# UCLALibrary/jp2-bucketeer

Hardware: AMD Instinct MI355X
Metric: encoded megapixels/sec (node), lossless 5/3 + lossy 9/7, at 1/2/4/8 MI355X (higher is better)
Workload: dtype f32+i32

## Files before the change

jp2-bucketeer_amd/csrc/encode.cpp:

```cpp
#include <algorithm>
#include <cmath>
#include <cstddef>
#include <cstring>
#include <string>
#include <vector>

#include "context.h"
#include "encode.h"
#include "source_layout.h"

namespace jp2hip {

void default_recipe(jp2hip_recipe *r, int conversion) {
    std::memset(r, 0, sizeof *r);
    r->levels = 6;
    r->layers = 6;
    r->tile_w = r->tile_h = 512;
    r->cblk_w_log2 = r->cblk_h_log2 = 6;
    r->nprecincts = 3;
    r->prec_w_log2[0] = r->prec_h_log2[0] = 8;
    r->prec_w_log2[1] = r->prec_h_log2[1] = 8;
    r->prec_w_log2[2] = r->prec_h_log2[2] = 7;
    r->progression = 2;
    r->sop = r->eph = r->plt = r->tparts_r = 1;
    r->guard_bits = 1;
    bool lossless = conversion == JP2HIP_LOSSLESS;
    r->reversible = lossless ? 1 : 0;
    r->mct = 1;
    r->qstep = 1.0 / 256.0;
    r->rate_bpp = lossless ? 0.0 : 3.0;
    r->format = JP2HIP_FORMAT_JPX;
    r->comment = 1;
    r->slope_skip = 1;
    r->flush_period = 1024;
}

jp2hip_recipe recipe_of(const jp2hip_recipe *recipe, int conversion) {
    jp2hip_recipe rc;
    std::memset(&rc, 0, sizeof rc);
    if (recipe) rc = *recipe;
    else default_recipe(&rc, conversion);
    const size_t gap0 = offsetof(jp2hip_recipe, mct) + sizeof rc.mct, gap1 = offsetof(jp2hip_recipe, qstep);
    if (gap1 > gap0) std::memset((char *)&rc + gap0, 0, gap1 - gap0);
    static_assert(offsetof(jp2hip_recipe, flush_period) + sizeof(int32_t) == sizeof(jp2hip_recipe),
                  "jp2hip_recipe: no tail padding");
    return rc;
}

namespace {

int64_t rate_target_of(const jp2hip_recipe &rc, int w, int h) {
    return (int64_t)std::floor(rc.rate_bpp * (double)w * (double)h / 8.0);
}
int64_t skip_target_of(const jp2hip_recipe &rc, int w, int h) {
    return rc.slope_skip && rc.rate_bpp > 0.0 ? rate_target_of(rc, w, h) : -1;
}
int64_t first_budget_of(const Plan &P, int64_t target) { return target - 16 * P.npackets - 16 * P.ntileparts - 256; }

int begin(jp2hip_ctx *ctx, const void *d_src, const jp2hip_layout *lay, int conversion, const jp2hip_recipe *recipe,
          const jp2hip_split *sp, jp2hip_recipe &rc, SourceMeta &meta, EncodeEnd &end) {
    if (conversion != JP2HIP_LOSSY && conversion != JP2HIP_LOSSLESS)
        return fail("conversion must be JP2HIP_LOSSY (0) or JP2HIP_LOSSLESS (1)");
    const int world = sp ? sp->world : 1, rank = sp ? sp->rank : 0;
    if (world < 1 || rank < 0 || rank >= world) return fail("split: bad rank / world");
    if (world > 1 && !sp->allreduce_sum) return fail("split: world > 1 needs an allreduce_sum callback");
    rc = recipe_of(recipe, conversion);
    if (!lay || !d_src) return fail("null source or layout");
    std::string terr;
    if (!resolve_tiles(rc, lay->width, lay->height, terr)) return fail(terr);
    meta = source_meta(*lay);
    ctx->gpu.take_waits();
    ctx->gpu.begin_encode();
    ctx->reused = ctx->ended;
    ctx->ended = 0;
    end.ctx = ctx;
    return 0;
}

struct FilePart {
    const Plan &file, &coded;
    bool with_main, with_eoc, have;
    size_t fh = 0, head = 0, bytes = 0;
    void size(const SourceMeta &meta, size_t mh_bytes, int64_t part_bytes) {
        fh = with_main ? file_header_bytes(file, meta) : 0;
        head = with_main ? fh + mh_bytes : 0;
        bytes = head + (size_t)(have ? part_bytes : 0) + (with_eoc ? 2 : 0);
    }
};

int finish_part(jp2hip_ctx *ctx, const FilePart &fp, const SourceMeta &meta, std::vector<uint64_t> K, int64_t tp_hdr,
                const int64_t *layer_bytes, int64_t cs_bytes, const T2Summary &sum, uint8_t *buf, StageTimes &st,
                uint8_t **out, size_t *out_len, jp2hip_stats *stats, double t_start, double h2d_ms,
                int64_t file_bytes, int iters) {
    const Plan &P = fp.file;
    std::string err;
    if (fp.with_main) {
        const int L = P.rc.layers;
        if (P.rc.rate_bpp <= 0.0) K[L - 1] = 0;
        std::vector<int64_t> layer_end((size_t)L);
        int64_t acc = (int64_t)(fp.head - fp.fh) + tp_hdr;
        for (int l = 0; l < L; l++) layer_end[l] = acc += layer_bytes[l];
        std::vector<uint8_t> mh;
        main_header(P, mh, K.data(), layer_end.data());
        write_file_header(P, meta, (uint64_t)cs_bytes, buf);
        std::memcpy(buf + fp.fh, mh.data(), mh.size());
    }
    const bool prof = ctx->cfg.profile != 0;
    if (fp.have && (!ctx->gpu.t2_emit(fp.coded, 0, (uint64_t)sum.part_bytes, buf + fp.head, prof, st, err) ||
                    !ctx->gpu.collect_profile(st, err))) {
        out_free(buf);
        return fail(err);
    }
    if (fp.with_eoc) {
        buf[fp.bytes - 2] = 0xFF;
        buf[fp.bytes - 1] = 0xD9;
    }
    *out = buf;
    *out_len = fp.bytes;
    if (!stats) return 0;
    std::memset(stats, 0, sizeof *stats);
    stats->total_ms = now_ms() - t_start;
    stats->h2d_ms = h2d_ms;
    stats->ingest_ms = st.ingest;
    stats->dwt_ms = st.dwt;
    stats->quant_ms = st.quant;
    stats->t1_ms = st.t1_cm + st.t1_mq;
    stats->t1_cm_ms = st.t1_cm;
    stats->t1_mq_ms = st.t1_mq;
    stats->pcrd_ms = st.pcrd;
    stats->d2h_ms = st.d2h;
    stats->t2_ms = st.t2;
    stats->codeblocks = (int64_t)fp.coded.blocks.size();
    stats->t1_bytes = sum.t1_bytes;
    stats->coded_passes = sum.coded_passes;
    stats->out_bytes = file_bytes;
    stats->rate_iterations = iters;
    stats->host_waits = ctx->gpu.take_waits();
    stats->mq_decisions = sum.decisions;
    stats->stream_need_bytes = sum.stream_need;
    stats->stream_pool_bytes = (int64_t)ctx->gpu.stream_pool_bytes();
    stats->pool_grows = ctx->gpu.take_pool_grows();
    stats->reused = ctx->reused | ctx->gpu.reuse_bits();
    return 0;
}

}

int encode_core(jp2hip_ctx *ctx, const void *d_src, size_t src_len, const jp2hip_layout *lay, int conversion,
                const jp2hip_recipe *recipe, uint8_t **out, size_t *out_len, jp2hip_stats *stats, double t_start,
                double h2d_ms) {
    jp2hip_recipe rc;
    SourceMeta meta;
    EncodeEnd end;
    if (begin(ctx, d_src, lay, conversion, recipe, nullptr, rc, meta, end)) return -1;
    std::string err;
    jp2hip_layout ulay;
    std::vector<uint64_t> uoffs;
    UnitGrid grid;
    if (!unit_grid(*lay, grid, err) || !prepare_source(ctx, grid, d_src, src_len, lay, 0, lay->height, ulay, uoffs, err))
        return fail(err);
    PlanCache &pc = ctx->pc;
    if (!pc.valid || pc.w != lay->width || pc.h != lay->height || pc.nc != lay->components || pc.bits != lay->bits ||
        std::memcmp(&pc.rc, &rc, sizeof rc) != 0) {
        pc.valid = false;
        if (!build_plan(pc.plan, rc, lay->width, lay->height, lay->components, lay->bits, err)) return fail(err);
        t2_tables(pc.plan, 0, pc.plan.ntx * pc.plan.nty, 0, pc.tabs);
        main_header(pc.plan, pc.mh0, nullptr, nullptr);
        pc.rc = rc;
        pc.w = lay->width; pc.h = lay->height; pc.nc = lay->components; pc.bits = lay->bits;
        pc.valid = true;
    } else {
        ctx->reused |= JP2HIP_REUSED_PLAN;
    }
    const Plan &plan = pc.plan;
    const bool prof = ctx->cfg.profile != 0;
    StageTimes st;
    int64_t skip_target = skip_target_of(rc, plan.w, plan.h);
    if (!ctx->gpu.t2_load(plan, pc.tabs, err)) return fail(err);
    if (!ctx->gpu.run_front(d_src, *lay, plan, prof, st, err, skip_target)) return fail(err);
    const size_t mh_bytes = pc.mh0.size();
    T2Summary sum;
    std::memset(&sum, 0, sizeof sum);
    int iters = 0;
    int64_t cs_bytes = 0;
    if (rc.rate_bpp <= 0.0) {
        for (int grow = 0;; grow++) {
            if (!ctx->gpu.select_lossless(plan, err) || !ctx->gpu.t2_size(plan, true, prof, st, sum, err))
                return fail(err);
            if ((sum.err & kErrSlotPool) && grow < 2) {
                if (!ctx->gpu.pool_grow(err) || !ctx->gpu.run_front(d_src, *lay, plan, prof, st, err, skip_target))
                    return fail(err);
                continue;
            }
            break;
        }
        if (sum.err) return fail("tier-1 output capacity exceeded");
        iters = 1;
        cs_bytes = (int64_t)mh_bytes + sum.part_bytes + 2;
    } else {
        RateState init;
        std::memset(&init, 0, sizeof init);
        init.target = rate_target_of(rc, plan.w, plan.h);
        init.budget = first_budget_of(plan, init.target);
        init.fixed = (int64_t)mh_bytes + 2;
        init.skip_target = skip_target;
        RateState rs;
        bool restart = true;
        for (int grow = 0;;) {
            if (!ctx->gpu.rate_loop(plan, init, restart, restart ? 1 : 2, prof, st, rs, sum, err)) return fail(err);
            restart = false;
            if ((sum.err & kErrSlotPool) && grow++ < 2) {
                if (!ctx->gpu.pool_grow(err) ||
                    !ctx->gpu.run_front(d_src, *lay, plan, prof, st, err, init.skip_target))
                    return fail(err);
                restart = true;
                continue;
            }
            if (sum.err) return fail("tier-1 output capacity exceeded");
            if (rs.safety) {
                init.skip_target = -1;
                if (!ctx->gpu.run_front(d_src, *lay, plan, prof, st, err, -1)) return fail(err);
                restart = true;
                continue;
            }
            if (rs.halt) break;
        }
        iters = rs.iters;
        cs_bytes = rs.cs_bytes;
    }
    FilePart fp{plan, plan, true, true, true};
    fp.size(meta, mh_bytes, sum.part_bytes);
    uint8_t *buf = out_alloc(fp.bytes);
    if (!buf) return fail("out of (pinned) host memory");
    if (finish_part(ctx, fp, meta, std::vector<uint64_t>(sum.kc, sum.kc + rc.layers), sum.tp_hdr_bytes,
                    sum.layer_bytes, cs_bytes, sum, buf, st, out, out_len, stats, t_start, h2d_ms, (int64_t)fp.bytes,
                    iters))
        return -1;
    end.ok = true;
    return 0;
}

int encode_split_core(jp2hip_ctx *ctx, const void *d_src, size_t src_len, const jp2hip_layout *lay, int conversion,
                      const jp2hip_recipe *recipe, const jp2hip_split *sp, uint8_t **out, size_t *out_len,
                      uint64_t *file_offset, uint64_t *file_len, jp2hip_stats *stats, double t_start) {
    jp2hip_recipe rc;
    SourceMeta meta;
    EncodeEnd end;
    if (begin(ctx, d_src, lay, conversion, recipe, sp, rc, meta, end)) return -1;
    const int world = sp ? sp->world : 1, rank = sp ? sp->rank : 0;
    std::string err;
    auto allreduce = [&](int64_t *v, int n) {
        return world <= 1 || sp->allreduce_sum(sp->user, v, (int32_t)n) == 0;
    };
    auto exchange = [&](std::vector<int64_t> &v, size_t flag, bool &ok) {
        v[flag] = ok ? 0 : 1;
        if (!allreduce(v.data(), (int)v.size())) {
            err = "split: all-reduce failed";
            return false;
        }
        if (ok && v[flag]) {
            ok = false;
            err = "split: another rank failed";
        }
        return true;
    };
    Plan full;
    UnitGrid grid;
    if (!unit_grid(*lay, grid, err)) return fail(err);
    int enc_nc, enc_bits;
    encoded_format(*lay, enc_nc, enc_bits);
    if (!build_plan(full, rc, lay->width, lay->height, enc_nc, enc_bits, err)) return fail(err);
    int tr0, tr1;
    if (untiled(recipe)) {
        tr0 = rank ? 1 : 0;
        tr1 = 1;
    } else {
        split_tile_rows(full.nty, rc.tile_h, full.h, rc.flush_period, rank, world, tr0, tr1);
    }
    Plan sub;
    make_subplan(full, tr0, tr1, sub);
    const bool have = sub.ntc > 0;
    jp2hip_layout ulay;
    std::vector<uint64_t> uoffs;
    bool ok = !have || prepare_source(ctx, grid, d_src, src_len, lay, sub.row0, sub.row0 + sub.band_h, ulay, uoffs, err);
    const bool prof = ctx->cfg.profile != 0;
    StageTimes st;
    std::vector<uint64_t> keys;
    std::vector<int64_t> cum;
    int64_t skip_target = skip_target_of(rc, full.w, full.h);
    bool hist_done = false;
    GpuEncoder::HistReduce reduce = [&](std::vector<int64_t> &h) {
        hist_done = true;
        std::vector<int64_t> v(h.size() + 1, 0);
        std::copy(h.begin(), h.end(), v.begin());
        bool all = true;
        if (!exchange(v, h.size(), all) || !all) return false;
        std::copy(v.begin(), v.end() - 1, h.begin());
        return true;
    };
    T2Tables tabs;
    const int tile0 = sub.tile0, tile1 = sub.tile0 + full.ntx * (tr1 - tr0);
    if (ok && have) {
        t2_tables(full, tile0, tile1, sub.block0, tabs);
        ok = ctx->gpu.t2_load(sub, tabs, err);
    }
    ok = ok && (!have || ctx->gpu.run_front(d_src, *lay, sub, prof, st, err, skip_target, &reduce, true));
    if (skip_target >= 0 && !hist_done) {
        std::vector<int64_t> v((size_t)kSlopeBins + 1, 0);
        if (!exchange(v, (size_t)kSlopeBins, ok)) return fail(err);
    }
    const int L = rc.layers;
    std::vector<int64_t> budgets((size_t)L, 0);
    std::vector<uint64_t> K((size_t)L);
    int iters = 0;
    int64_t cs_bytes = 0;
    T2Summary sum;
    std::memset(&sum, 0, sizeof sum);
    int64_t g_tp_hdr = 0;
    std::vector<int64_t> g_layer((size_t)L, 0);
    std::vector<uint8_t> mh;
    main_header(full, mh, nullptr, nullptr);
    auto round = [&](bool lossless) -> bool {
        if (!lossless && jp2hip_split_thresholds(keys.data(), cum.data(), (int64_t)keys.size(), budgets.data(), L, sp,
                                                 K.data()) != 0) {
            err = "split: threshold exchange failed";
            return false;
        }
        bool rok = ok;
        if (rok && have)
            rok = (lossless ? ctx->gpu.select_lossless(sub, err) : ctx->gpu.select_keys(sub, K, err)) &&
                  ctx->gpu.t2_size(sub, lossless, prof, st, sum, err);
        if (rok && have && sum.err) {
            rok = false;
            err = "tier-1 output capacity exceeded";
        }
        std::vector<int64_t> v((size_t)L + 3 + (lossless ? (size_t)world * L : 0), 0);
        if (rok && have) {
            v[0] = sum.part_bytes;
            v[2] = sum.tp_hdr_bytes;
            for (int l = 0; l < L; l++) {
                v[3 + l] = sum.layer_bytes[l];
                if (lossless) v[3 + L + (size_t)rank * L + l] = (int64_t)sum.kc[l];
            }
        }
        if (!exchange(v, 1, rok) || !rok) return false;
        cs_bytes = (int64_t)mh.size() + 2 + v[0];
        g_tp_hdr = v[2];
        g_layer.assign(v.begin() + 3, v.begin() + 3 + L);
        iters++;
        for (int l = 0; lossless && l < L; l++) {
            K[l] = 0;
            for (int r = 0; r < world; r++) K[l] = std::max(K[l], (uint64_t)v[3 + L + (size_t)r * L + l]);
        }
        return true;
    };
    for (int attempt = 0; attempt < 2; attempt++) {
        if (attempt == 1) {
            keys.clear();
            cum.clear();
            ok = !have || ctx->gpu.run_front(d_src, *lay, sub, prof, st, err, -1, nullptr, true);
            skip_target = -1;
            iters = 0;
        }
        if (rc.rate_bpp <= 0.0) {
            if (!round(true)) return fail(err);
            break;
        }
        ok = ok && (!have || ctx->gpu.segments(sub, keys, cum, err));
        std::vector<int64_t> flag(1);
        if (!exchange(flag, 0, ok) || !ok) return fail(err);
        const int64_t target = rate_target_of(rc, full.w, full.h);
        int64_t budget = first_budget_of(full, target);
        bool rerun = false;
        for (int it = 0; it < 8; it++) {
            if (budget < 0) budget = 0;
            for (int l = 0; l < L; l++) budgets[l] = budget >> (L - 1 - l);
            if (!round(false)) return fail(err);
            if (it == 0 && skip_target > 0) {
                int64_t v[2] = {have ? sum.t1_bytes : 0, have ? sum.skipped : 0};
                if (!allreduce(v, 2)) return fail("split: all-reduce failed");
                if (v[1] && v[0] < skip_target) { rerun = true; break; }
            }
            if (cs_bytes <= target) break;
            budget -= ((cs_bytes - target) << it) + ((cs_bytes - target) >> 4) + 64;
        }
        if (!rerun) break;
    }
    FilePart fp{full, sub, rank == 0, rank == world - 1, have};
    fp.size(meta, mh.size(), sum.part_bytes);
    uint8_t *buf = out_alloc(fp.bytes);
    bool ready = buf != nullptr;
    if (!ready) err = "out of (pinned) host memory";
    if (ready && have) ready = ctx->gpu.t2_reserve(sum.part_bytes, err);
    std::vector<int64_t> sizes((size_t)world + 1, 0);
    sizes[rank] = (int64_t)fp.bytes;
    if (!exchange(sizes, (size_t)world, ready) || !ready) {
        out_free(buf);
        return fail(err);
    }
    uint64_t off = 0, flen = 0;
    for (int r = 0; r < world; r++) {
        if (r < rank) off += (uint64_t)sizes[r];
        flen += (uint64_t)sizes[r];
    }
    if (finish_part(ctx, fp, meta, K, g_tp_hdr, g_layer.data(), cs_bytes, sum, buf, st, out, out_len, stats, t_start,
                    0.0, (int64_t)flen, iters))
        return -1;
    if (file_offset) *file_offset = off;
    if (file_len) *file_len = flen;
    end.ok = true;
    return 0;
}

}
```

jp2-bucketeer_amd/csrc/gpu_encoder.cpp:

```cpp
#include <algorithm>
#include <atomic>
#include <chrono>
#include <cstdio>
#include <cstdlib>
#include <cstring>
#include <string>
#include <thread>
#include <vector>

#include "gpu_encoder.h"
#include "hip_check.h"

namespace jp2hip {

static std::atomic<long long> g_test_held{0};
static long long test_device_bytes() {
    static const long long v = [] {
        const char *s = getenv("JP2HIP_TEST_DEVICE_BYTES");
        return s ? atoll(s) : 0ll;
    }();
    return v;
}

hipError_t GpuEncoder::device_alloc(void **p, size_t n) {
    const long long cap = test_device_bytes();
    if (cap > 0) {
        if (g_test_held.fetch_add((long long)n) + (long long)n > cap) {
            g_test_held.fetch_sub((long long)n);
            return hipErrorOutOfMemory;
        }
        const hipError_t e = hipMalloc(p, n);
        if (e != hipSuccess) g_test_held.fetch_sub((long long)n);
        return e;
    }
    return hipMalloc(p, n);
}

void GpuEncoder::device_free(DevBuf &b) {
    if (b.ptr) {
        (void)hipFree(b.ptr);
        if (test_device_bytes() > 0) g_test_held.fetch_sub((long long)b.bytes);
    }
    held -= b.bytes;
    b.ptr = nullptr;
    b.bytes = 0;
}

bool GpuEncoder::trim(size_t soft) {
    if (held <= soft) return false;
    for (DevBuf *b : bufs()) device_free(*b);
#ifdef JP2HIP_DEBUG_DUMPS
    if (held != 0) {
        fprintf(stderr, "jp2hip: trim: %zu bytes still accounted after every buffer was freed\n", held);
        abort();
    }
#endif
    front_gen = 0;
    t2_gen = 0;
    strips_dev = nullptr;
    strips_host.clear();
    dma_ok = false;
    pool_hint = 0;
    return true;
}

bool GpuEncoder::pool_grow(std::string &err) {
    unsigned long long used = 0;
    HIPCHECK(hipStreamSynchronize(stream));
    HIPCHECK(hipMemcpy(&used, (unsigned long long *)mqspan.ptr + 2, sizeof used, hipMemcpyDeviceToHost));
    pool_hint = std::max<uint64_t>(pool_hint, used + used / 8);
    pool_grows++;
    return true;
}

void GpuEncoder::quiesce() {
    if (stream) (void)hipStreamSynchronize(stream);
    (void)hipGetLastError();
}

GpuEncoder::~GpuEncoder() {
    for (DevBuf *b : bufs()) device_free(*b);
    if (sync_ev) (void)hipEventDestroy(sync_ev);
    if (stg_ev) (void)hipEventDestroy(stg_ev);
    for (const PinnedChunk &c : stg) (void)hipHostFree(c.p);
    if (stream) (void)hipStreamDestroy(stream);
    for (int i = 0; i < kNumEvents; i++)
        if (ev[i]) (void)hipEventDestroy(ev[i]);
    if (h_sum) (void)hipHostFree(h_sum);
    if (h_tot) (void)hipHostFree(h_tot);
    if (h_rs) (void)hipHostFree(h_rs);
    if (dma_dep.handle) (void)hsa_signal_destroy(dma_dep);
    if (dma_done.handle) (void)hsa_signal_destroy(dma_done);
    if (hsa_up) (void)hsa_shut_down();
}

bool GpuEncoder::init(int dev, std::string &err) {
    device = dev;
    if (const char *f = getenv("JP2HIP_TEST_POOL_FRAC")) pool_frac_test = atof(f);
    HIPCHECK(hipSetDevice(dev));
    HIPCHECK(hipStreamCreateWithFlags(&stream, hipStreamNonBlocking));
    for (int i = 0; i < kNumEvents; i++) HIPCHECK(hipEventCreate(&ev[i]));
    HIPCHECK(hipEventCreateWithFlags(&sync_ev, hipEventBlockingSync | hipEventDisableTiming));
    HIPCHECK(hipEventCreateWithFlags(&stg_ev, hipEventDisableTiming));
    HIPCHECK(hipHostMalloc((void **)&h_tot, 8 * sizeof(int64_t), hipHostMallocDefault));
    return true;
}

bool GpuEncoder::check_residency(std::string &err) {
    hipDevice_t sd = -1;
    HIPCHECK(hipStreamGetDevice(stream, &sd));
    if ((int)sd != device) {
        err = "context on device " + std::to_string(device) + ": its stream is on device " + std::to_string((int)sd);
        return false;
    }
    const DevBuf *bufs[] = {&src, &coef, &bp, &t1out, &stream_buf, &t2out, &blocks};
    for (const DevBuf *b : bufs) {
        if (!b->ptr) continue;
        hipPointerAttribute_t at;
        HIPCHECK(hipPointerGetAttributes(&at, b->ptr));
        if (at.device != device) {
            err = "context on device " + std::to_string(device) + ": a buffer lives on device " +
                  std::to_string(at.device);
            return false;
        }
    }
    return true;
}

bool GpuEncoder::h2d(void *dst, const void *src, size_t bytes, std::string &err) {
    if (!bytes) return true;
    if (hipEventQuery(stg_ev) == hipSuccess) {
        if (stg.size() > 1) {
            size_t tot = 0;
            for (const PinnedChunk &c : stg) {
                tot += c.cap;
                HIPCHECK(hipHostFree(c.p));
            }
            stg.clear();
            PinnedChunk c{nullptr, tot};
            HIPCHECK(hipHostMalloc((void **)&c.p, tot, hipHostMallocDefault));
            stg.push_back(c);
        }
        stg_used = 0;
    }
    const size_t need = (bytes + 255) & ~(size_t)255;
    if (stg.empty() || stg_used + need > stg.back().cap) {
        PinnedChunk c{nullptr, std::max<size_t>(need, stg.empty() ? (size_t)1 << 20 : 2 * stg.back().cap)};
        HIPCHECK(hipHostMalloc((void **)&c.p, c.cap, hipHostMallocDefault));
        stg.push_back(c);
        stg_used = 0;
    }
    uint8_t *h = stg.back().p + stg_used;
    stg_used += need;
    std::memcpy(h, src, bytes);
    HIPCHECK(hipMemcpyAsync(dst, h, bytes, hipMemcpyHostToDevice, stream));
    HIPCHECK(hipEventRecord(stg_ev, stream));
    return true;
}

#ifndef JP2HIP_WAIT_POLL_US
#define JP2HIP_WAIT_POLL_US 0
#endif
bool GpuEncoder::host_wait(std::string &err) {
    waits++;
    HIPCHECK(hipEventRecord(sync_ev, stream));
#if JP2HIP_WAIT_POLL_US > 0
    for (;;) {
        const hipError_t q = hipEventQuery(sync_ev);
        if (q == hipSuccess) break;
        if (q != hipErrorNotReady) HIPCHECK(q);
        std::this_thread::sleep_for(std::chrono::microseconds(JP2HIP_WAIT_POLL_US));
    }
#else
    HIPCHECK(hipEventSynchronize(sync_ev));
#endif
    return true;
}

bool GpuEncoder::upload_source(const void *host, size_t len, std::string &err) {
    HIPCHECK(hipSetDevice(device));
    if (!ensure<uint8_t>(src, len, err)) return false;
    HIPCHECK(hipMemcpyAsync(src.ptr, host, len, hipMemcpyHostToDevice, stream));
    return true;
}

bool GpuEncoder::dump(const char *dir, const char *name, const DevBuf &b, size_t bytes,
                      std::string &err) {
    std::vector<uint8_t> h(bytes);
    if (!host_wait(err)) return false;
    if (bytes) HIPCHECK(hipMemcpy(h.data(), b.ptr, bytes, hipMemcpyDeviceToHost));
    std::string path = std::string(dir) + "/" + name;
    FILE *f = fopen(path.c_str(), "wb");
    if (!f) { err = "cannot write dump " + path; return false; }
    fwrite(h.data(), 1, bytes, f);
    fclose(f);
    return true;
}

bool GpuEncoder::collect_profile(StageTimes &st, std::string &err) {
    if (!profiled || !h_tot) return true;
    float t;
    HIPCHECK(hipEventElapsedTime(&t, ev[kEvFrontBegin], ev[kEvDwtBegin])); st.ingest = t;
    if (expand_timed) {
        HIPCHECK(hipEventElapsedTime(&t, ev[kEvExpandBegin], ev[kEvExpandEnd]));
        st.ingest += t;
    }
    HIPCHECK(hipEventElapsedTime(&t, ev[kEvDwtBegin], ev[kEvDwtEnd])); st.dwt = t;
    HIPCHECK(hipEventElapsedTime(&t, ev[kEvDwtEnd], ev[kEvQuantEnd])); st.quant = t;
    HIPCHECK(hipEventElapsedTime(&t, ev[kEvCmBegin], ev[kEvCmEnd])); st.t1_cm = t;
    HIPCHECK(hipEventElapsedTime(&t, ev[kEvCmEnd], ev[kEvMqEnd])); st.t1_mq = t;
    HIPCHECK(hipEventElapsedTime(&t, ev[kEvMqEnd], ev[kEvHullEnd])); st.pcrd += t;
    return true;
}

}
```

jp2-bucketeer_amd/csrc/gpu_encoder.h:

```cpp
#pragma once

#include <hip/hip_runtime.h>
#include <hsa/hsa.h>
#include <hsa/hsa_ext_amd.h>

#include <array>
#include <chrono>
#include <cstdint>
#include <functional>
#include <string>
#include <thread>
#include <vector>

#include "jp2hip_internal.h"
#include "source_layout.h"
#include "stages.h"

namespace jp2hip {

struct DevBuf {
    void *ptr = nullptr;
    size_t bytes = 0;
    size_t want = 0;
};

struct StageTimes {
    double ingest = 0, dwt = 0, quant = 0, t1_cm = 0, t1_mq = 0, pcrd = 0, d2h = 0, t2 = 0;
};

struct T2Args;
struct FrontJob;

#define JP2HIP_DEVBUFS(X)                                                                                     \
    X(coef) X(blocks) X(order) X(bp) X(sm) X(P) X(dref) X(dsig) X(t1out) X(rates) X(dists) X(npasses)         \
    X(lengths) X(weight) X(nhull) X(hpass) X(hkey) X(budget) X(nl) X(lrate) X(err) X(tcw) X(tch) X(strips)    \
    X(src) X(segcnt) X(segoff) X(est) X(hist) X(pmin) X(mqspan) X(stage) X(soff) X(lzwseg) X(untiled)         \
    X(inflnk) X(segkey) X(llbuf0) X(llbuf1) X(ordkey) X(segval) X(thr) X(items) X(slotoff) X(stream_buf)      \
    X(counts) X(dspp) X(dbgbuf) X(t1fill) X(dbgsel)                                                           \
          \
    X(pcrd_hb) X(pcrd_hc) X(sel_ctl) X(sel_key) X(sel_size)                                                   \
            \
                                                                                   \
    X(grptab) X(gtot)                                                                                         \
                                                                           \
    X(hdist) X(rstate) X(t2ticket) X(t2prec) X(t2tp) X(t2tt) X(t2lblock) X(t2incl) X(t2pklen) X(t2pkoff)      \
    X(t2tplen) X(t2tphdr) X(t2tpoff) X(t2blkdst) X(t2out) X(t2sum) X(t2seq)                                   \
               \
    X(expanded) X(exoff) X(exlut)

class GpuEncoder {
  public:
    ~GpuEncoder();
    bool init(int device, std::string &err);

    size_t device_bytes() const { return held; }
    void set_limits(size_t soft, size_t hard) {
        mem_soft = soft;
        mem_hard = hard;
    }
    size_t soft_limit() const { return mem_soft; }
    size_t hard_limit() const { return mem_hard; }
    bool trim(size_t soft);
    void begin_encode() {
        for (DevBuf *b : bufs()) b->want = 0;
        expand_timed = false;
        reuse = 0;
        reuse_front_noted = false;
    }
    int reuse_bits() const { return reuse; }
    size_t need_bytes() {
        size_t n = 0;
        for (DevBuf *b : bufs()) n += b->want;
        return n;
    }
    std::function<bool()> reclaim;
    void quiesce();
    template <typename T>
    bool ensure(DevBuf &b, size_t count, std::string &err);

    bool upload_source(const void *host, size_t len, std::string &err);
    const void *source() const { return src.ptr; }
    bool unpack_strips(const void *d_src, const jp2hip_layout &lay, const UnitGrid &g, jp2hip_layout &out,
                       std::vector<uint64_t> &out_offs, const void **d_out, std::string &err, bool untile = true);

    bool expand_samples(const void *d_src, const jp2hip_layout &lay, const UnitGrid &g, const uint32_t *lut,
                        bool profile, const void **d_out, std::string &err);

    using HistReduce = std::function<bool(std::vector<int64_t> &)>;
    bool run_front(const void *d_src, const jp2hip_layout &lay, const Plan &plan, bool profile,
                   StageTimes &st, std::string &err, int64_t skip_target = -1,
                   const HistReduce *reduce = nullptr, bool pool_worst = false);
    bool pool_grow(std::string &err);
    size_t stream_pool_bytes() const { return stream_buf.bytes; }
    int take_pool_grows() {
        const int g = pool_grows;
        pool_grows = 0;
        return g;
    }
    bool select_lossless(const Plan &plan, std::string &err);
    bool select_keys(const Plan &plan, const std::vector<uint64_t> &K, std::string &err);
    bool t2_load(const Plan &plan, const T2Tables &T, std::string &err);
    bool t2_size(const Plan &plan, bool with_kc, bool profile, StageTimes &st, T2Summary &sum, std::string &err);
    bool rate_loop(const Plan &plan, const RateState &init, bool restart, int batch, bool profile, StageTimes &st,
                   RateState &rs, T2Summary &sum, std::string &err);
    bool t2_reserve(uint64_t part_bytes, std::string &err);
    bool t2_emit(const Plan &plan, uint64_t base, uint64_t part_bytes, uint8_t *host_dst, bool profile,
                 StageTimes &st, std::string &err);
    bool collect_profile(StageTimes &st, std::string &err);
    bool segments(const Plan &plan, std::vector<uint64_t> &keys, std::vector<int64_t> &cum, std::string &err);
    hipStream_t get_stream() const { return stream; }
    int get_device() const { return device; }
    bool check_residency(std::string &err);
    int take_waits() {
        const int w = waits;
        waits = 0;
        return w;
    }

  private:
    bool dump(const char *dir, const char *name, const DevBuf &b, size_t bytes, std::string &err);
    bool front_reserve(FrontJob &j, std::string &err);
    bool front_upload(const FrontJob &j, std::string &err);
    bool front_first_args(FrontJob &j, std::string &err);
    bool front_ingest_dwt(const FrontJob &j, std::string &err);
    bool front_quant(const FrontJob &j, std::string &err);
    bool front_predict_items(const FrontJob &j, std::string &err);
    bool front_t1(const FrontJob &j, std::string &err);
    bool hull_launch(const Plan &plan, std::string &err);
    bool front_dumps(const FrontJob &j, std::string &err);
    bool apply_thresholds(const Plan &plan, const int *halt, std::string &err);
    void select_launch(const Plan &plan, const int *halt, const RateState *init = nullptr, RateState *rs = nullptr);
    T2Args t2_args(const Plan &plan) const;
    void t2_size_launch(const Plan &plan, bool with_kc, const int *halt, RateState *rs = nullptr,
                        RateState *out_rs = nullptr);
    bool host_wait(std::string &err);
    bool dma_init(std::string &err);
    bool dma_to_host(uint8_t *host_dst, const void *src, size_t bytes, std::string &err);
    hsa_signal_t dma_dep{0}, dma_done{0};
    volatile hsa_signal_value_t *dma_dep_val = nullptr;
    hsa_agent_t dma_gpu{0}, dma_cpu{0};
    int dma_engine = -1;
    bool dma_ok = false, hsa_up = false;
    bool h2d(void *dst, const void *src, size_t bytes, std::string &err);
    struct PinnedChunk {
        uint8_t *p;
        size_t cap;
    };
    std::vector<PinnedChunk> stg;
    size_t stg_used = 0;
    hipEvent_t stg_ev = nullptr;
    enum Ev {
        kEvFrontBegin,
        kEvDwtBegin,
        kEvDwtEnd,
        kEvQuantEnd,
        kEvCmBegin,
        kEvCmEnd,
        kEvMqEnd,
        kEvHullEnd,
        kEvSelectBegin,
        kEvSelectEnd,
        kEvT2Begin,
        kEvT2End,
        kEvExpandBegin,
        kEvExpandEnd,
        kNumEvents
    };
    int device = 0;
    int waits = 0;
    hipEvent_t sync_ev = nullptr;
    hipStream_t stream = nullptr;
    hipEvent_t ev[kNumEvents] = {};
#define X(name) DevBuf name;
    JP2HIP_DEVBUFS(X)
#undef X
    RateState *h_rs = nullptr;
    RateState *d_rs_out = nullptr;
    int t2_nprec = 0, t2_ntp = 0;
    bool t2_wave = true;
    bool t2_seq = false;
    uint64_t front_gen = 0, t2_gen = 0;
    int reuse = 0;
    bool reuse_front_noted = false;
    T2Summary *h_sum = nullptr;
    int64_t *h_tot = nullptr;
    bool profiled = false;
    bool expand_timed = false;
    int nseg = 0;
    std::vector<int64_t> h_hist;
    std::vector<uint64_t> strips_host;
    const void *strips_dev = nullptr;
    size_t held = 0, mem_soft = SIZE_MAX, mem_hard = SIZE_MAX;
    static constexpr int kReclaimWaitMs = 30000;
    hipError_t device_alloc(void **p, size_t n);
    void device_free(DevBuf &b);
    static constexpr double kPoolFracLossy = 0.3, kPoolFracLossless = 0.7;
    uint64_t pool_hint = 0;
    int pool_grows = 0;
    double pool_frac_test = -1.0;
#define X(name) +1
    static constexpr int kNumBufs = 0 JP2HIP_DEVBUFS(X);
#undef X
#define X(name) &name,
    std::array<DevBuf *, kNumBufs> bufs() { return {{JP2HIP_DEVBUFS(X)}}; }
#undef X
};

template <typename T>
bool GpuEncoder::ensure(DevBuf &b, size_t count, std::string &err) {
    size_t bytes = count * sizeof(T);
    if (bytes == 0) bytes = 16;
    if (bytes > b.want) b.want = bytes;
    if (b.bytes >= bytes) return true;
    const size_t alloc = bytes + bytes / 8;
    if (held - b.bytes + alloc > mem_hard) {
        err = "device memory limit: this image needs a " + std::to_string(alloc) + "-byte buffer, the context holds " +
              std::to_string(held) + " of its " + std::to_string(mem_hard) + " bytes";
        return false;
    }
    device_free(b);
    hipError_t e = device_alloc(&b.ptr, alloc);
    for (int waited = 0; e == hipErrorOutOfMemory && reclaim && waited <= kReclaimWaitMs; waited += 5) {
        (void)hipGetLastError();
        if (!reclaim()) std::this_thread::sleep_for(std::chrono::milliseconds(5));
        e = device_alloc(&b.ptr, alloc);
    }
    if (e != hipSuccess) {
        (void)hipGetLastError();
        b.ptr = nullptr;
        err = std::string("hipMalloc(") + std::to_string(alloc) + "): " + hipGetErrorString(e);
        return false;
    }
    b.bytes = alloc;
    held += alloc;
    return true;
}

}
```

jp2-bucketeer_amd/csrc/jp2hip_internal.h:

```cpp
#pragma once

#include <cstdint>
#include <string>
#include <vector>

#include "jp2hip.h"

namespace jp2hip {

constexpr int kMaxPasses = 96;
constexpr int kSlopeBins = 1024;
constexpr int kSlopeBinBase = (1023 - 64) << 3;
constexpr int kSkipMargin = 12;
constexpr int kPcrdBins = 4096;
constexpr int kPcrdBinBase = (1023 - 64) << 5;
constexpr int kMaxLayers = 32;
constexpr int kMaxLevels = 12;

struct BandQuant {
    int eps = 0, mu = 0, Mb = 0;
    float inv_delta = 1.0f;
    double wnorm = 1.0;
};

BandQuant band_quant(const jp2hip_recipe &rc, int bits, int level, int band);

struct QuantTab {
    float inv[kMaxLevels + 1][4];
    uint32_t lim[kMaxLevels + 1][4];
    int q16;
};
QuantTab quant_tab(const jp2hip_recipe &rc, int bits);

constexpr int kErrSlotPool = 8;

struct BlockDesc {
    int32_t tc;
    int16_t x0, y0;
    int16_t w, h;
    int8_t band;
    int8_t Mb;
    int8_t pad0, pad1;
    float inv_delta;
    uint32_t pad2;
    uint64_t bp_off;
    uint64_t sm_off;
    uint64_t out_off;
    uint32_t out_cap;
    uint32_t pad3;
};
static_assert(sizeof(BlockDesc) == 56, "BlockDesc layout");

struct PrecBand {
    int ncw = 0, nch = 0;
    int first = 0;
};
struct Precinct {
    PrecBand pb[3];
    int nb = 0;
};
struct Resolution {
    int npx = 0, npy = 0;
    std::vector<Precinct> prec;
};
struct TileComp {
    Resolution res[kMaxLevels + 1];
};
struct Tile {
    int tx0, ty0, tx1, ty1;
    std::vector<TileComp> tc;
};

struct Plan {
    jp2hip_recipe rc;
    int w = 0, h = 0, nc = 0, bits = 0;
    int ntx = 0, nty = 0, ntc = 0;
    int plane_w = 0, plane_h = 0;
    std::vector<Tile> tiles;
    std::vector<BlockDesc> blocks;
    std::vector<double> weight;
    std::vector<int32_t> t1_order;
    std::vector<int32_t> tc_w, tc_h;
    uint64_t bp_words = 0, sm_words = 0, out_bytes = 0;
    int64_t npackets = 0, ntileparts = 0;
    double compw[4] = {1, 1, 1, 1};
    int row0 = 0, band_h = 0, tile0 = 0, block0 = 0;
    std::vector<int32_t> tile_b0;
    std::vector<int32_t> grp_b0;
    int ngroups() const { return (int)grp_b0.size() - 1; }
    uint64_t gen = 0;
};

bool build_plan(Plan &plan, const jp2hip_recipe &rc, int w, int h, int nc, int bits,
                std::string &err);
constexpr int kMaxTileSide = 32768;
bool resolve_tiles(jp2hip_recipe &rc, int w, int h, std::string &err);
inline bool untiled(const jp2hip_recipe *rc) { return rc && rc->tile_w == 0 && rc->tile_h == 0; }

int prec_log2(const jp2hip_recipe &rc, int r, bool vertical);

int32_t lossless_layer_frac(int l, int NL);

std::vector<int> flush_stripe_ends(int nty, int tile_h, int h, int period);
void split_tile_rows(int nty, int tile_h, int h, int period, int rank, int world, int &tr0, int &tr1);
void make_subplan(const Plan &full, int tr0, int tr1, Plan &sub);

struct PrecDesc {
    int32_t first[3];
    uint16_t ncw[3], nch[3];
    int32_t tt_off;
    int32_t nsop0;
    uint8_t nb, pad0;
    uint16_t nsop_step;
};
static_assert(sizeof(PrecDesc) == 36, "PrecDesc layout");
struct TpDesc {
    int32_t tile, tpsot, tnsot;
    int32_t prec0, nprec;
};
struct T2Tables {
    std::vector<PrecDesc> prec;
    std::vector<TpDesc> tp;
    std::vector<uint32_t> seq;
    int64_t tt_nodes = 0;
    int max_prec_blocks = 0;
};
void t2_tables(const Plan &P, int tile0, int tile1, int block0, T2Tables &T);
void packet_sequence(const Plan &P, int t, std::vector<uint32_t> &seq);
struct T2Summary {
    int64_t part_bytes;
    int64_t tp_hdr_bytes;
    int64_t layer_bytes[kMaxLayers];
    uint64_t kc[kMaxLayers];
    int64_t t1_bytes, coded_passes;
    int64_t decisions;
    int32_t skipped, err;
    int64_t stream_need;
};
struct RateState {
    int64_t budget, target, fixed, skip_target, cs_bytes;
    int32_t it, halt, safety, iters;
};
void main_header(const Plan &P, std::vector<uint8_t> &v, const uint64_t *K, const int64_t *layer_end);

struct SourceMeta {
    int32_t extra_samples = 0, res_unit = 0;
    uint32_t xres_num = 0, xres_den = 0, yres_num = 0, yres_den = 0;
    const uint8_t *icc = nullptr;
    uint64_t icc_bytes = 0;
};
SourceMeta source_meta(const jp2hip_layout &lay);

int classify_icc(const uint8_t *icc, uint64_t n, int nc, uint32_t *embed);

size_t file_header_bytes(const Plan &plan, const SourceMeta &meta);
void write_file_header(const Plan &plan, const SourceMeta &meta, uint64_t cs_bytes, uint8_t *dst);

}
```

jp2-bucketeer_amd/csrc/t2.cpp:

```cpp
#include <algorithm>
#include <cmath>
#include <cstdio>
#include <cstring>
#include <numeric>

#include "jp2hip_internal.h"

namespace jp2hip {

namespace {

inline void be16(uint8_t *p, uint32_t v) { p[0] = (uint8_t)(v >> 8); p[1] = (uint8_t)v; }
inline void be32(uint8_t *p, uint32_t v) {
    p[0] = (uint8_t)(v >> 24); p[1] = (uint8_t)(v >> 16); p[2] = (uint8_t)(v >> 8); p[3] = (uint8_t)v;
}

}

static constexpr char kComVersion[] = "jp2hip-v0.2.0";
static constexpr char kLayerHdr[] = "Kdu-Layer-Info: log_2{Delta-D(squared-error)/Delta-L(bytes)}, L(bytes)\n";

static double layer_log_slope(uint64_t K, int bits) {
    if (K == 0) return -192.0;
    if (K >= 0x7FF0000000000000ull) return 192.0;
    double s;
    std::memcpy(&s, &K, 8);
    const double v = std::log2(s) - 2.0 * bits;
    return v < -192.0 ? -192.0 : (v > 192.0 ? 192.0 : v);
}

void main_header(const Plan &P, std::vector<uint8_t> &v, const uint64_t *K, const int64_t *layer_end) {
    const jp2hip_recipe &rc = P.rc;
    const int L = rc.levels, nc = P.nc;
    v.clear();
    auto u8 = [&](int x) { v.push_back((uint8_t)x); };
    auto u16 = [&](int x) { u8(x >> 8); u8(x); };
    auto u32 = [&](uint32_t x) { u16((int)(x >> 16)); u16((int)(x & 0xFFFF)); };
    auto raw = [&](const char *p, size_t n) { v.insert(v.end(), p, p + n); };
    u16(0xFF4F);
    u16(0xFF51);
    u16(38 + 3 * nc);
    u16(0);
    u32((uint32_t)P.w); u32((uint32_t)P.h);
    u32(0); u32(0);
    u32((uint32_t)rc.tile_w); u32((uint32_t)rc.tile_h);
    u32(0); u32(0);
    u16(nc);
    for (int c = 0; c < nc; c++) { u8(P.bits - 1); u8(1); u8(1); }
    u16(0xFF52);
    u16(12 + L + 1);
    u8(0x01 | (rc.sop ? 2 : 0) | (rc.eph ? 4 : 0));
    u8(rc.progression);
    u16(rc.layers);
    u8((rc.mct && nc >= 3) ? 1 : 0);
    u8(L);
    u8(rc.cblk_w_log2 - 2);
    u8(rc.cblk_h_log2 - 2);
    u8(0);
    u8(rc.reversible ? 1 : 0);
    for (int r = 0; r <= L; r++) u8((prec_log2(rc, r, true) << 4) | prec_log2(rc, r, false));
    u16(0xFF5C);
    const int nbands = 3 * L + 1;
    u16(3 + (rc.reversible ? nbands : 2 * nbands));
    u8((rc.guard_bits << 5) | (rc.reversible ? 0 : 2));
    for (int i = 0; i < nbands; i++) {
        const int d = (i == 0) ? L : L - (i - 1) / 3;
        const int band = (i == 0) ? 0 : 1 + (i - 1) % 3;
        const BandQuant q = band_quant(rc, P.bits, d, band);
        if (rc.reversible) u8(q.eps << 3);
        else u16((q.eps << 11) | q.mu);
    }
    if (rc.comment) {
        const size_t nv = sizeof kComVersion - 1, nh = sizeof kLayerHdr - 1;
        u16(0xFF64);
        u16(4 + (int)nv);
        u16(1);
        raw(kComVersion, nv);
        u16(0xFF64);
        u16(4 + (int)nh + 17 * rc.layers);
        u16(1);
        raw(kLayerHdr, nh);
        for (int l = 0; l < rc.layers; l++) {
            char line[64];
            const int n = std::snprintf(line, sizeof line, "%6.1f, %8.1e\n", K ? layer_log_slope(K[l], P.bits) : 0.0,
                                        layer_end ? (double)layer_end[l] : 0.0);
            if (n != 17) {
                std::memset(line, ' ', 16);
                line[16] = '\n';
            }
            raw(line, 17);
        }
    }
}

static int64_t tree_nodes(int w, int h) {
    int64_t n = 0;
    for (;;) {
        n += (int64_t)w * h;
        if (w == 1 && h == 1) return n;
        w = (w + 1) / 2;
        h = (h + 1) / 2;
    }
}

void packet_sequence(const Plan &P, int t, std::vector<uint32_t> &seq) {
    const jp2hip_recipe &rc = P.rc;
    const int Lv = rc.levels, L = rc.layers, order = rc.progression;
    const Tile &Tl = P.tiles[(size_t)t];
    struct Prec {
        int32_t r, c, raster;
        int64_t x, y;
        uint32_t p;
    };
    std::vector<Prec> pv;
    for (int r = 0; r <= Lv; r++) {
        const Resolution &R0 = Tl.tc[0].res[r];
        if (R0.npx * R0.npy == 0) continue;
        const int sh = Lv - r, ppx = prec_log2(rc, r, false), ppy = prec_log2(rc, r, true);
        const int64_t px0 = ((int64_t)Tl.tx0 >> sh) >> ppx, py0 = ((int64_t)Tl.ty0 >> sh) >> ppy;
        for (int py = 0; py < R0.npy; py++)
            for (int px = 0; px < R0.npx; px++)
                for (int c = 0; c < P.nc; c++) {
                    Prec e;
                    e.r = r;
                    e.c = c;
                    e.raster = py * R0.npx + px;
                    e.x = std::max<int64_t>(Tl.tx0, (px0 + px) << (ppx + sh));
                    e.y = std::max<int64_t>(Tl.ty0, (py0 + py) << (ppy + sh));
                    e.p = (uint32_t)pv.size();
                    pv.push_back(e);
                }
    }
    seq.clear();
    seq.reserve(pv.size() * (size_t)L);
    if (order == JP2HIP_ORDER_LRCP || order == JP2HIP_ORDER_RLCP) {
        std::stable_sort(pv.begin(), pv.end(), [](const Prec &a, const Prec &b) {
            return a.r != b.r ? a.r < b.r : (a.c != b.c ? a.c < b.c : a.raster < b.raster);
        });
        if (order == JP2HIP_ORDER_LRCP) {
            for (int l = 0; l < L; l++)
                for (const Prec &e : pv) seq.push_back(e.p * (uint32_t)L + (uint32_t)l);
        } else {
            for (size_t i = 0; i < pv.size();) {
                size_t j = i;
                while (j < pv.size() && pv[j].r == pv[i].r) j++;
                for (int l = 0; l < L; l++)
                    for (size_t k = i; k < j; k++) seq.push_back(pv[k].p * (uint32_t)L + (uint32_t)l);
                i = j;
            }
        }
        return;
    }
    if (order == JP2HIP_ORDER_PCRL)
        std::stable_sort(pv.begin(), pv.end(), [](const Prec &a, const Prec &b) {
            return a.y != b.y ? a.y < b.y : (a.x != b.x ? a.x < b.x : (a.c != b.c ? a.c < b.c : a.r < b.r));
        });
    else if (order == JP2HIP_ORDER_CPRL)
        std::stable_sort(pv.begin(), pv.end(), [](const Prec &a, const Prec &b) {
            return a.c != b.c ? a.c < b.c : (a.y != b.y ? a.y < b.y : (a.x != b.x ? a.x < b.x : a.r < b.r));
        });
    for (const Prec &e : pv)
        for (int l = 0; l < L; l++) seq.push_back(e.p * (uint32_t)L + (uint32_t)l);
}

void t2_tables(const Plan &P, int tile0, int tile1, int block0, T2Tables &T) {
    const jp2hip_recipe &rc = P.rc;
    const int Lv = rc.levels, L = rc.layers;
    const bool resequence = rc.progression != JP2HIP_ORDER_RPCL;
    std::vector<uint32_t> tseq, pos;
    T.prec.clear();
    T.tp.clear();
    T.seq.clear();
    T.tt_nodes = 0;
    T.max_prec_blocks = 0;
    std::vector<std::vector<TpDesc>> per_tile((size_t)std::max(0, tile1 - tile0));
    for (int t = tile0; t < tile1; t++) {
        const Tile &Tl = P.tiles[t];
        int nsop = 0;
        const size_t tile_prec0 = T.prec.size();
        std::vector<TpDesc> &tps = per_tile[(size_t)(t - tile0)];
        for (int r = 0; r <= Lv; r++) {
            const Resolution &R0 = Tl.tc[0].res[r];
            if (R0.npx * R0.npy == 0) continue;
            if (rc.tparts_r || tps.empty()) tps.push_back(TpDesc{t, (int32_t)tps.size(), 0, (int32_t)T.prec.size(), 0});
            TpDesc &tp = tps.back();
            for (int py = 0; py < R0.npy; py++)
                for (int px = 0; px < R0.npx; px++)
                    for (int c = 0; c < P.nc; c++) {
                        const Precinct &pr = Tl.tc[c].res[r].prec[(size_t)py * R0.npx + px];
                        PrecDesc d;
                        std::memset(&d, 0, sizeof d);
                        d.nb = (uint8_t)pr.nb;
                        d.tt_off = (int32_t)T.tt_nodes;
                        d.nsop0 = nsop;
                        d.nsop_step = 1;
                        int blocks = 0;
                        for (int bi = 0; bi < pr.nb; bi++) {
                            const PrecBand &pb = pr.pb[bi];
                            d.first[bi] = pb.first - block0;
                            d.ncw[bi] = (uint16_t)pb.ncw;
                            d.nch[bi] = (uint16_t)pb.nch;
                            blocks += pb.ncw * pb.nch;
                            if (pb.ncw && pb.nch) T.tt_nodes += 2 * tree_nodes(pb.ncw, pb.nch);
                        }
                        T.max_prec_blocks = std::max(T.max_prec_blocks, blocks);
                        T.prec.push_back(d);
                        tp.nprec++;
                        nsop += L;
                    }
        }
        for (TpDesc &tp : tps) tp.tnsot = (&tp == &tps.back()) ? (int32_t)tps.size() : 0;
        if (resequence) {
            packet_sequence(P, t, tseq);
            pos.resize(tseq.size());
            for (size_t s = 0; s < tseq.size(); s++) pos[tseq[s]] = (uint32_t)s;
            for (size_t i = tile_prec0; i < T.prec.size(); i++) {
                const size_t k = (i - tile_prec0) * (size_t)L;
                T.prec[i].nsop0 = (int32_t)pos[k];
                T.prec[i].nsop_step = L > 1 ? (uint16_t)(pos[k + 1] - pos[k]) : 1;
            }
            const uint32_t base = (uint32_t)(tile_prec0 * (size_t)L);
            for (uint32_t s : tseq) T.seq.push_back(base + s);
        }
    }
    const std::vector<int> ends = flush_stripe_ends(P.nty, rc.tile_h, P.h, rc.flush_period);
    int ty0 = 0;
    for (int e : ends) {
        const int a = std::max(tile0, ty0 * P.ntx), b = std::min(tile1, e * P.ntx);
        for (int k = 0; k <= Lv; k++)
            for (int t = a; t < b; t++) {
                const std::vector<TpDesc> &tps = per_tile[(size_t)(t - tile0)];
                if (k < (int)tps.size()) T.tp.push_back(tps[(size_t)k]);
            }
        ty0 = e;
    }
}


SourceMeta source_meta(const jp2hip_layout &lay) {
    SourceMeta m;
    m.extra_samples = lay.extra_samples;
    m.res_unit = lay.res_unit;
    m.xres_num = lay.xres_num; m.xres_den = lay.xres_den;
    m.yres_num = lay.yres_num; m.yres_den = lay.yres_den;
    if (lay.icc && lay.icc_bytes) { m.icc = lay.icc; m.icc_bytes = lay.icc_bytes; }
    return m;
}

namespace {

inline uint32_t rd32(const uint8_t *p) {
    return ((uint32_t)p[0] << 24) | ((uint32_t)p[1] << 16) | ((uint32_t)p[2] << 8) | p[3];
}
inline bool sig_is(const uint8_t *p, const char *s) { return std::memcmp(p, s, 4) == 0; }

constexpr uint64_t kMaxIccBytes = 0xFFFFFFFFull - 1024;

struct Resc {
    uint32_t n = 0, d = 0;
    int e = 0;
};

bool resc_axis(uint32_t num, uint32_t den, int unit, Resc &r) {
    if (!num || !den || (unit != 2 && unit != 3)) return false;
    uint64_t P = (uint64_t)num * (unit == 2 ? 10000 : 100), Q = (uint64_t)den * (unit == 2 ? 254 : 1);
    const uint64_t g = std::gcd(P, Q);
    P /= g;
    Q /= g;
    if (P <= 65535 && Q <= 65535) {
        r.n = (uint32_t)P; r.d = (uint32_t)Q; r.e = 0;
        return true;
    }
    typedef unsigned __int128 u128;
    for (int E = -20; E <= 20; E++) {
        u128 A = P, B = Q;
        for (int k = 0; k < (E < 0 ? -E : E); k++) (E < 0 ? A : B) *= 10;
        const u128 N = (2 * A + B) / (2 * B);
        if (N > 65535) continue;
        if (N < 6554) return false;
        r.n = (uint32_t)N; r.d = 1; r.e = E;
        return true;
    }
    return false;
}

struct HeaderBoxes {
    bool enum_colr = true;
    int meth = 0;
    uint32_t icc_len = 0;
    int cdef_typ = -1;
    bool res = false;
    Resc v, h;
    uint32_t jp2h = 0;
};

HeaderBoxes header_boxes(const Plan &P, const SourceMeta &m) {
    HeaderBoxes b;
    const int nc = P.nc;
    uint32_t embed = 0;
    const int cls = classify_icc(m.icc, m.icc_bytes, nc, &embed);
    if (cls == 1) {
        b.enum_colr = false;
        b.meth = 2;
    } else if (cls == 2 && P.rc.format == JP2HIP_FORMAT_JPX) {
        b.meth = 3;
    }
    b.icc_len = b.meth ? embed : 0;
    if (nc == 4 || nc == 2) {
        b.cdef_typ = m.extra_samples == 1 ? -1 : (m.extra_samples == 2 ? 2 : 1);
    }
    b.res = resc_axis(m.yres_num, m.yres_den, m.res_unit, b.v) && resc_axis(m.xres_num, m.xres_den, m.res_unit, b.h);
    b.jp2h = 8 + (8 + 14) + (b.enum_colr ? 8 + 7 : 0) + (b.meth ? 8 + 3 + b.icc_len : 0) +
             (b.cdef_typ >= 0 ? (uint32_t)(8 + 2 + 6 * nc) : 0) + (b.res ? 8 + (8 + 10) : 0);
    return b;
}

}

int classify_icc(const uint8_t *icc, uint64_t n, int nc, uint32_t *embed) {
    *embed = 0;
    if (!icc || n < 132) return 0;
    const uint64_t S = rd32(icc);
    if (S < 132 || S > n || S > kMaxIccBytes) return 0;
    if (!sig_is(icc + 36, "acsp")) return 0;
    const bool rgb = nc >= 3;
    if (!sig_is(icc + 16, rgb ? "RGB " : "GRAY")) return 0;
    *embed = (uint32_t)S;
    if (!sig_is(icc + 12, "scnr") && !sig_is(icc + 12, "mntr")) return 2;
    if (!sig_is(icc + 20, "XYZ ")) return 2;
    const uint64_t ntags = rd32(icc + 128);
    if (132 + 12 * ntags > S) return 2;
    static const char *const kRgbTags[] = {"rXYZ", "gXYZ", "bXYZ", "rTRC", "gTRC", "bTRC"};
    static const char *const kGrayTags[] = {"kTRC"};
    const char *const *need = rgb ? kRgbTags : kGrayTags;
    const int nneed = rgb ? 6 : 1;
    unsigned have = 0;
    for (uint64_t i = 0; i < ntags; i++) {
        const uint8_t *t = icc + 132 + 12 * i;
        if (sig_is(t, "A2B0")) return 2;
        for (int k = 0; k < nneed; k++)
            if (sig_is(t, need[k])) have |= 1u << k;
    }
    return have == (1u << nneed) - 1 ? 1 : 2;
}

size_t file_header_bytes(const Plan &P, const SourceMeta &meta) {
    if (P.rc.format == JP2HIP_FORMAT_J2K) return 0;
    size_t n = 12;
    n += (P.rc.format == JP2HIP_FORMAT_JPX) ? (8 + 4 + 4 + 12) + (8 + 10) : (8 + 4 + 4 + 4);
    n += header_boxes(P, meta).jp2h;
    return n + 8;
}

void write_file_header(const Plan &P, const SourceMeta &meta, uint64_t cs_bytes, uint8_t *dst) {
    if (P.rc.format == JP2HIP_FORMAT_J2K) return;
    uint8_t *p = dst;
    auto raw = [&](const void *s, size_t n) { std::memcpy(p, s, n); p += n; };
    auto u8 = [&](int x) { *p++ = (uint8_t)x; };
    auto u16 = [&](int x) { be16(p, (uint32_t)x); p += 2; };
    auto u32 = [&](uint32_t x) { be32(p, x); p += 4; };
    auto box = [&](uint32_t len, const char *type) { u32(len); raw(type, 4); };
    static const uint8_t sig[12] = {0, 0, 0, 12, 'j', 'P', ' ', ' ', 0x0D, 0x0A, 0x87, 0x0A};
    raw(sig, 12);
    const int nc = P.nc;
    if (P.rc.format == JP2HIP_FORMAT_JPX) {
        box(8 + 4 + 4 + 12, "ftyp");
        raw("jpx ", 4); u32(0);
        raw("jpx ", 4); raw("jp2 ", 4); raw("jpxb", 4);
        box(8 + 10, "rreq");
        u8(1); u8(0x80); u8(0x80);
        u16(1); u16(5); u8(0x80);
        u16(0);
    } else {
        box(8 + 4 + 4 + 4, "ftyp");
        raw("jp2 ", 4); u32(0); raw("jp2 ", 4);
    }
    const HeaderBoxes hb = header_boxes(P, meta);
    box(hb.jp2h, "jp2h");
    box(8 + 14, "ihdr");
    u32((uint32_t)P.h); u32((uint32_t)P.w);
    u16(nc); u8(P.bits - 1); u8(7); u8(0); u8(0);
    if (hb.enum_colr) {
        box(8 + 7, "colr");
        u8(1); u8(0); u8(0);
        u32(nc >= 3 ? 16 : 17);
    }
    if (hb.meth) {
        box(8 + 3 + hb.icc_len, "colr");
        u8(hb.meth);
        u8(hb.meth == 3 ? 1 : 0);
        u8(hb.meth == 3 ? 1 : 0);
        raw(meta.icc, hb.icc_len);
    }
    if (hb.cdef_typ >= 0) {
        box((uint32_t)(8 + 2 + 6 * nc), "cdef");
        u16(nc);
        for (int c = 0; c < nc; c++) {
            const bool alpha = (c == nc - 1);
            u16(c); u16(alpha ? hb.cdef_typ : 0); u16(alpha ? 0 : c + 1);
        }
    }
    if (hb.res) {
        box(8 + (8 + 10), "res ");
        box(8 + 10, "resc");
        u16((int)hb.v.n); u16((int)hb.v.d); u16((int)hb.h.n); u16((int)hb.h.d);
        u8(hb.v.e); u8(hb.h.e);
    }
    box(8 + cs_bytes > 0xFFFFFFFFull ? 0u : (uint32_t)(8 + cs_bytes), "jp2c");
}

}
```

jp2-bucketeer_amd/csrc/t2_device.hip:

```cpp
#include <hip/hip_runtime.h>

#include <algorithm>
#include <atomic>
#include <chrono>
#include <cstdio>
#include <cstring>
#include <map>
#include <memory>
#include <mutex>
#include <string>
#include <vector>

#include "device_common.h"
#include "gpu_encoder.h"
#include "hip_check.h"
#include "host_wait.h"
#include "stage_repeat.h"

namespace jp2hip {

struct T2Args {
    const PrecDesc *prec;
    int nprec;
    const TpDesc *tps;
    int ntp;
    const BlockDesc *blocks;
    const uint8_t *P;
    uint8_t *nl;
    int32_t *lrate;
    const uint8_t *nhull, *hpass, *npasses;
    const uint64_t *hkey, *K;
    const int32_t *grp_b0;
    int ngroups;
    const int32_t *rates;
    int lossless;
    int L, sop, eph, plt;
    uint32_t *tt;
    int8_t *lblock, *incl;
    uint32_t *pk_len;
    const uint32_t *seq;
    uint32_t *tp_len;
    uint32_t *tp_hdr;
    uint64_t *tp_off;
    uint64_t *pk_off;
    uint64_t *blkdst;
    uint8_t *out;
    uint64_t base;
    const int *halt;
};

template <bool EMIT>
struct DevBits {
    uint8_t *p;
    uint32_t nbytes;
    uint64_t acc;
    int n, cap;
    __device__ __forceinline__ void init(uint8_t *dst) { p = dst; nbytes = 0; acc = 0; n = 0; cap = 8; }
    __device__ __forceinline__ void put(uint32_t val, int nb) {
        acc = (acc << nb) | val;
        n += nb;
        while (n >= cap) {
            n -= cap;
            const uint32_t byte = (uint32_t)(acc >> n) & ((1u << cap) - 1u);
            if (EMIT) p[nbytes] = (uint8_t)byte;
            nbytes++;
            cap = (byte == 0xFF) ? 7 : 8;
        }
    }
    __device__ __forceinline__ void bit(int b) { put((uint32_t)(b & 1), 1); }
    __device__ __forceinline__ void flush() {
        if (n) {
            const uint32_t byte = (uint32_t)(acc << (cap - n)) & ((1u << cap) - 1u);
            if (EMIT) p[nbytes] = (uint8_t)byte;
            nbytes++;
        } else if (cap == 7) {
            if (EMIT) p[nbytes] = 0;
            nbytes++;
        }
        cap = 8;
        n = 0;
        acc = 0;
    }
};

__device__ __forceinline__ int tree_size(int w, int h) {
    int n = 0;
    for (;;) {
        n += w * h;
        if (w == 1 && h == 1) return n;
        w = (w + 1) >> 1;
        h = (h + 1) >> 1;
    }
}

__device__ __forceinline__ void tree_set(uint32_t *nd, int w, int h, int leaf, int v) {
    int x = leaf % w, y = leaf / w, base = 0;
    for (;;) {
        uint32_t &e = nd[base + y * w + x];
        if ((int)(e & 0xFFu) <= v) return;
        e = (e & ~0xFFu) | (uint32_t)v;
        if (w == 1 && h == 1) return;
        base += w * h;
        w = (w + 1) >> 1;
        h = (h + 1) >> 1;
        x >>= 1;
        y >>= 1;
    }
}

template <bool EMIT>
__device__ __forceinline__ void tree_encode(uint32_t *nd, int w, int h, int leaf, int threshold, DevBits<EMIT> &bw) {
    const int lx = leaf % w, ly = leaf / w;
    int nlev = 1;
    for (int cw = w, ch = h; cw != 1 || ch != 1; cw = (cw + 1) >> 1, ch = (ch + 1) >> 1) nlev++;
    int low = 0;
    for (int k = nlev - 1; k >= 0; k--) {
        int base = 0, cw = w, ch = h;
        for (int j = 0; j < k; j++) {
            base += cw * ch;
            cw = (cw + 1) >> 1;
            ch = (ch + 1) >> 1;
        }
        uint32_t &e = nd[base + (ly >> k) * cw + (lx >> k)];
        const int value = (int)(e & 0xFFu);
        int nlow = (int)((e >> 8) & 0xFFu);
        bool known = (e >> 16) & 1u;
        if (low > nlow) nlow = low;
        else low = nlow;
        const int nz = max(0, min(value, threshold) - low);
        low += nz;
        const bool one = low < threshold && !known;
        if (one) known = true;
        const int nb = nz + (one ? 1 : 0);
        if (nb > 32) {
            bw.put(0u, nb - 32);
            bw.put(one ? 1u : 0u, 32);
        } else if (nb > 0) {
            bw.put(one ? 1u : 0u, nb);
        }
        e = (uint32_t)value | ((uint32_t)low << 8) | (known ? (1u << 16) : 0u);
    }
}

__device__ __forceinline__ int dev_floor_log2(int v) { return 31 - __clz(v); }

constexpr int kLdsNodes = 48;

template <bool EMIT>
__global__ void __launch_bounds__(64) k_t2_code(T2Args a) {
    __shared__ uint32_t lds_nodes[64 * kLdsNodes];
    const int pi = blockIdx.x * 64 + threadIdx.x;
    if (pi >= a.nprec || (!EMIT && a.halt && *a.halt)) return;
    const PrecDesc d = a.prec[pi];
    const int L = a.L;
    int nodes = 0;
#pragma unroll
    for (int bi = 0; bi < 3; bi++)
        if (bi < d.nb && d.ncw[bi] && d.nch[bi]) nodes += 2 * tree_size(d.ncw[bi], d.nch[bi]);
    uint32_t *tt = nodes <= kLdsNodes ? lds_nodes + threadIdx.x * kLdsNodes : a.tt + d.tt_off;
    for (int i = 0; i < nodes; i++) tt[i] = 0xFFu;
    int toff[3];
    {
        int o = 0;
#pragma unroll
        for (int bi = 0; bi < 3; bi++) {
            toff[bi] = o;
            if (bi < d.nb && d.ncw[bi] && d.nch[bi]) o += 2 * tree_size(d.ncw[bi], d.nch[bi]);
        }
    }
#pragma unroll
    for (int bi = 0; bi < 3; bi++) {
        const int w = bi < d.nb ? d.ncw[bi] : 0, h = bi < d.nb ? d.nch[bi] : 0;
        if (!w || !h) continue;
        uint32_t *ti = tt + toff[bi], *tz = ti + tree_size(w, h);
        for (int k = 0; k < w * h; k++) {
            const int b = d.first[bi] + k;
            a.lblock[b] = 3;
            a.incl[b] = -1;
            const uint8_t *nb = a.nl + (size_t)b * L;
            int first = L;
            for (int l = 0; l < L; l++)
                if (nb[l] > 0) { first = l; break; }
            tree_set(ti, w, h, k, first);
            tree_set(tz, w, h, k, a.blocks[b].Mb - a.P[b]);
        }
    }
    const uint32_t fixed = (a.sop ? 6u : 0u) + (a.eph ? 2u : 0u);
    for (int l = 0; l < L; l++) {
        const size_t pk = (size_t)pi * L + l;
        bool nonempty = false;
#pragma unroll
        for (int bi = 0; bi < 3; bi++) {
            const int nk = bi < d.nb ? d.ncw[bi] * d.nch[bi] : 0;
            for (int k = 0; k < nk && !nonempty; k++) {
                const uint8_t *nb = a.nl + (size_t)(d.first[bi] + k) * L;
                if (nb[l] > (l ? nb[l - 1] : 0)) nonempty = true;
            }
        }
        uint8_t *o = nullptr;
        if (EMIT) {
            o = a.out + a.pk_off[pk];
            if (a.sop) {
                const uint32_t ns = (uint32_t)(d.nsop0 + l * (int)d.nsop_step) & 0xFFFFu;
                o[0] = 0xFF; o[1] = 0x91; o[2] = 0; o[3] = 4; o[4] = (uint8_t)(ns >> 8); o[5] = (uint8_t)ns;
                o += 6;
            }
        }
        DevBits<EMIT> w;
        w.init(o);
        w.bit(nonempty ? 1 : 0);
        uint32_t body = 0;
        if (nonempty) {
#pragma unroll
            for (int bi = 0; bi < 3; bi++) {
                const int cw = bi < d.nb ? d.ncw[bi] : 0, ch = bi < d.nb ? d.nch[bi] : 0;
                if (!cw || !ch) continue;
                uint32_t *ti = tt + toff[bi], *tz = ti + tree_size(cw, ch);
                for (int k = 0; k < cw * ch; k++) {
                    const int b = d.first[bi] + k;
                    const uint8_t *nb = a.nl + (size_t)b * L;
                    const int n = nb[l] - (l ? nb[l - 1] : 0);
                    const bool first_time = a.incl[b] < 0;
                    if (first_time) tree_encode(ti, cw, ch, k, l + 1, w);
                    else w.bit(n > 0 ? 1 : 0);
                    if (n <= 0) continue;
                    if (first_time) {
                        tree_encode(tz, cw, ch, k, 1 << 20, w);
                        a.incl[b] = (int8_t)l;
                    }
                    if (n == 1) w.bit(0);
                    else if (n == 2) w.put(2u, 2);
                    else if (n <= 5) w.put((3u << 2) | (uint32_t)(n - 3), 4);
                    else if (n <= 36) w.put((15u << 5) | (uint32_t)(n - 6), 9);
                    else w.put((511u << 7) | (uint32_t)(n - 37), 16);
                    const int32_t *lr = a.lrate + (size_t)b * L;
                    const int r0 = l ? lr[l - 1] : 0;
                    const int len = lr[l] - r0;
                    int lb = a.lblock[b];
                    int nbits = lb + dev_floor_log2(n);
                    while (len >= (1 << nbits)) { w.bit(1); lb++; nbits++; }
                    a.lblock[b] = (int8_t)lb;
                    w.bit(0);
                    w.put((uint32_t)len, nbits);
                    if (EMIT) a.blkdst[(size_t)b * L + l] = body;
                    body += (uint32_t)len;
                }
            }
        }
        w.flush();
        if (EMIT) {
            o += w.nbytes;
            if (a.eph) { o[0] = 0xFF; o[1] = 0x92; o += 2; }
            const uint64_t at = (uint64_t)(o - a.out);
            if (nonempty)
#pragma unroll
                for (int bi = 0; bi < 3; bi++) {
                    const int nk = bi < d.nb ? d.ncw[bi] * d.nch[bi] : 0;
                    for (int k = 0; k < nk; k++) {
                        const int b = d.first[bi] + k;
                        const uint8_t *nb = a.nl + (size_t)b * L;
                        if (nb[l] > (l ? nb[l - 1] : 0)) a.blkdst[(size_t)b * L + l] += at;
                    }
                }
        } else {
            a.pk_len[pk] = fixed + w.nbytes + body;
        }
    }
}

constexpr int kT2Waves = 4;
constexpr int kTreeLev = 7;
constexpr int kBitWords = 512;
constexpr int kWaveMaxMb = 48;
struct T2LaneShared {
    int32_t *lr;
    uint32_t *bits;
    uint8_t *nl;
};
__host__ __device__ constexpr size_t t2_lane_bytes(int L) {
    return ((size_t)L * 64 * 5 + (size_t)kBitWords * 4 + 15) & ~(size_t)15;
}
__device__ __forceinline__ T2LaneShared t2_lane(uint8_t *dyn, int L, int wv) {
    uint8_t *p = dyn + (size_t)wv * t2_lane_bytes(L);
    T2LaneShared S;
    S.lr = (int32_t *)p;
    S.bits = (uint32_t *)(p + (size_t)L * 64 * 4);
    S.nl = p + (size_t)L * 64 * 4 + (size_t)kBitWords * 4;
    return S;
}

__device__ __forceinline__ void wave_lds_sync() {
    __builtin_amdgcn_wave_barrier();
    asm volatile("" ::: "memory");
}

__device__ __forceinline__ void lds_put_bits(uint32_t *buf, uint32_t p, uint64_t v, int nb) {
    if (nb <= 0) return;
    const uint64_t x = v << (64 - nb);
    const int sh = (int)(p & 31u);
    uint32_t *w = buf + (p >> 5);
    const uint64_t hi = x >> sh;
    const uint32_t w0 = (uint32_t)(hi >> 32), w1 = (uint32_t)hi, w2 = sh ? (uint32_t)((x << (64 - sh)) >> 32) : 0u;
    if (w0) atomicOr(w, w0);
    if (w1) atomicOr(w + 1, w1);
    if (w2) atomicOr(w + 2, w2);
}

template <bool EMIT>
__device__ __forceinline__ uint32_t stuff_header(const uint32_t *buf, uint32_t p0, uint32_t nbits, uint8_t *o) {
    uint32_t q = 0, nbytes = 0, byte = 0;
    int cap = 8;
    while (q < nbits) {
        const uint32_t p = p0 + q;
        const uint64_t win = ((uint64_t)buf[p >> 5] << 32) | buf[(p >> 5) + 1];
        byte = (uint32_t)(win >> (64 - cap - (int)(p & 31u))) & ((1u << cap) - 1u);
        if (EMIT) o[nbytes] = (uint8_t)byte;
        nbytes++;
        q += (uint32_t)cap;
        cap = byte == 0xFFu ? 7 : 8;
    }
    if (byte == 0xFFu) {
        if (EMIT) o[nbytes] = 0;
        nbytes++;
    }
    return nbytes;
}

template <bool EMIT>
__device__ __forceinline__ void t2_wave_precinct(const T2Args &a, const T2LaneShared &S, int pi) {
    const int lane = threadIdx.x & 63;
    const PrecDesc d = a.prec[pi];
    const int L = a.L;
    const int c0 = d.nb > 0 ? d.ncw[0] * d.nch[0] : 0, c1 = d.nb > 1 ? d.ncw[1] * d.nch[1] : 0,
              c2 = d.nb > 2 ? d.ncw[2] * d.nch[2] : 0;
    const int nbt = c0 + c1 + c2;
    const bool own = lane < nbt;
    const int bi = lane < c0 ? 0 : (lane < c0 + c1 ? 1 : 2);
    const int leaf = own ? lane - (bi == 0 ? 0 : (bi == 1 ? c0 : c0 + c1)) : 0;
    const int bfirst = bi == 0 ? d.first[0] : (bi == 1 ? d.first[1] : d.first[2]);
    const int bcw = bi == 0 ? d.ncw[0] : (bi == 1 ? d.ncw[1] : d.ncw[2]);
    const int bch = bi == 0 ? d.nch[0] : (bi == 1 ? d.nch[1] : d.nch[2]);
    const int b = own ? bfirst + leaf : 0;
    int zero_planes = 0;
    if (own) {
        zero_planes = a.blocks[b].Mb - a.P[b];
        uint8_t *gnl = a.nl + (size_t)b * L;
        int32_t *glr = a.lrate + (size_t)b * L;
        if (!EMIT) {
            const int nh = a.nhull[b];
            const uint8_t *hp = a.hpass + (size_t)b * (kMaxPasses + 1);
            const uint64_t *hk = a.hkey + (size_t)b * (kMaxPasses + 1);
            const int32_t *R = a.rates + (size_t)b * kMaxPasses;
            const uint64_t *Kb = a.K + (size_t)block_group(a.grp_b0, a.ngroups, b) * kMaxLayers;
            uint64_t k8[8];
#pragma unroll
            for (int i = 0; i < 8; i++) k8[i] = hk[min(i, kMaxPasses)];
            int at = 0;
            auto key = [&](int i) {
                uint64_t r = 0;
#pragma unroll
                for (int t = 0; t < 8; t++) r = i == t ? k8[t] : r;
                return i < 8 ? r : hk[i];
            };
            for (int l0 = 0; l0 < L; l0 += 8) {
                int atv[8];
#pragma unroll
                for (int j = 0; j < 8; j++) {
                    const int l = l0 + j;
                    if (l < L && !(a.lossless && l == L - 1)) {
                        const uint64_t K = Kb[l];
                        while (at + 1 < nh && key(at + 1) >= K) at++;
                        while (at > 0 && key(at) < K) at--;
                    }
                    atv[j] = at;
                }
                int ncv[8];
#pragma unroll
                for (int j = 0; j < 8; j++) {
                    const int l = l0 + j;
                    ncv[j] = (a.lossless && l == L - 1) ? (int)a.npasses[b] : (int)hp[atv[j]];
                }
                int32_t rv[8];
#pragma unroll
                for (int j = 0; j < 8; j++) rv[j] = R[max(ncv[j], 1) - 1];
#pragma unroll
                for (int j = 0; j < 8; j++) {
                    const int l = l0 + j;
                    if (l >= L) break;
                    const int32_t r = ncv[j] ? rv[j] : 0;
                    S.nl[l * 64 + lane] = (uint8_t)ncv[j];
                    S.lr[l * 64 + lane] = r;
                    gnl[l] = (uint8_t)ncv[j];
                    glr[l] = r;
                }
            }
        } else {
            for (int l = 0; l < L; l++) {
                S.nl[l * 64 + lane] = gnl[l];
                S.lr[l * 64 + lane] = glr[l];
            }
        }
    }
    int firstl = L;
    if (own)
        for (int l = 0; l < L; l++)
            if (S.nl[l * 64 + lane] > 0) {
                firstl = l;
                break;
            }
    const int cw0 = own ? bcw : 1, ch0 = own ? bch : 1;
    const int lx = leaf % cw0, ly = leaf / cw0;
    int nlev = 1;
    for (int w = cw0, h = ch0; w != 1 || h != 1; w = (w + 1) >> 1, h = (h + 1) >> 1) nlev++;
    const int key = (bi << 16) | (ly << 8) | lx;
    uint64_t imask[kTreeLev];
    int ival[kTreeLev], zval[kTreeLev], zbest[kTreeLev];
#pragma unroll
    for (int k = 0; k < kTreeLev; k++) {
        imask[k] = 0;
        ival[k] = L;
        zval[k] = 255;
        zbest[k] = 0x7FFFFFFF;
    }
    for (int j = 0; j < nbt; j++) {
        const int kj = __builtin_amdgcn_readlane(key, j);
        const int fj = __builtin_amdgcn_readlane(firstl, j), zj = __builtin_amdgcn_readlane(zero_planes, j);
        const int xj = kj & 0xFF, yj = (kj >> 8) & 0xFF;
        const bool band = (kj >> 16) == bi;
#pragma unroll
        for (int k = 0; k < kTreeLev; k++)
            if (band && (xj >> k) == (lx >> k) && (yj >> k) == (ly >> k)) {
                imask[k] |= 1ull << j;
                ival[k] = min(ival[k], fj);
                zval[k] = min(zval[k], zj);
                if (fj < L) zbest[k] = min(zbest[k], (fj << 6) | j);
            }
    }
    const int myz = (firstl << 6) | lane;
    const uint64_t below = (1ull << lane) - 1ull;
    uint32_t *buf = S.bits;
    for (int i = lane; i < kBitWords; i += 64) buf[i] = 0;
    wave_lds_sync();
    int lb = 3;
    const uint32_t fixed = (a.sop ? 6u : 0u) + (a.eph ? 2u : 0u);
    uint32_t used = 0, pws = 0, pnb = 0, pbody = 0;
    int l0 = 0;
    int tp = 0;
    for (int l = 0; l <= L; l++) {
        int n = 0, len = 0;
        uint64_t I = 0, Z = 0, p1v = 0;
        int nI = 0, nZ = 0, p1n = 0, p2n = 0;
        uint32_t nbits = 0, need = 0, off = 0, body = 0;
        if (l < L) {
            if (own) {
                n = (int)S.nl[l * 64 + lane] - (l ? (int)S.nl[(l - 1) * 64 + lane] : 0);
                len = S.lr[l * 64 + lane] - (l ? S.lr[(l - 1) * 64 + lane] : 0);
            }
            if (n > 0) {
                uint32_t cv;
                int cn;
                if (n == 1) { cv = 0u; cn = 1; }
                else if (n == 2) { cv = 2u; cn = 2; }
                else if (n <= 5) { cv = (3u << 2) | (uint32_t)(n - 3); cn = 4; }
                else if (n <= 36) { cv = (15u << 5) | (uint32_t)(n - 6); cn = 9; }
                else { cv = (511u << 7) | (uint32_t)(n - 37); cn = 16; }
                const int nbits0 = lb + dev_floor_log2(n);
                const int bl = len > 0 ? 32 - __clz(len) : 0;
                const int extra = bl > nbits0 ? bl - nbits0 : 0;
                lb += extra;
                p1v = ((uint64_t)cv << (extra + 1)) | (((1ull << extra) - 1ull) << 1);
                p1n = cn + extra + 1;
                p2n = lb + dev_floor_log2(n);
            }
            const bool nonempty = __ballot(n > 0) != 0ull;
            const bool visitor = own && firstl >= l;
            const uint64_t vis = __ballot(visitor);
            if (nonempty && own) {
                if (visitor) {
#pragma unroll
                    for (int k = kTreeLev - 1; k >= 0; k--) {
                        if (k >= nlev || (imask[k] & vis & below)) continue;
                        const int v = ival[k], pv = k + 1 < nlev ? ival[k + 1 < kTreeLev ? k + 1 : k] : 0;
                        const int nz = max(0, min(v, l + 1) - max(min(v, tp), min(pv, l + 1)));
                        const int one = (v >= tp && v <= l) ? 1 : 0;
                        I = (I << (nz + one)) | (uint64_t)one;
                        nI += nz + one;
                    }
                    if (n > 0)
#pragma unroll
                        for (int k = kTreeLev - 1; k >= 0; k--) {
                            if (k >= nlev || zbest[k] != myz) continue;
                            const int z = zval[k] - (k + 1 < nlev ? zval[k + 1 < kTreeLev ? k + 1 : k] : 0);
                            Z = (Z << (z + 1)) | 1u;
                            nZ += z + 1;
                        }
                } else {
                    I = n > 0 ? 1u : 0u;
                    nI = 1;
                }
            }
            if (nonempty) tp = l + 1;
            const uint32_t T = (uint32_t)(nI + nZ + p1n + p2n);
            off = wave_incl_scan(T) - T;
            nbits = 1u + (uint32_t)__shfl((int)(off + T), 63, 64);
            const uint32_t lin = n > 0 ? (uint32_t)len : 0u;
            body = (uint32_t)__shfl((int)wave_incl_scan(lin), 63, 64);
            need = (nbits + 31u) / 32u + 1u;
            if (!nonempty) nbits = 1;
        }
        if (l == L || used + need > (uint32_t)kBitWords) {
            wave_lds_sync();
            uint32_t hdr = 0;
            if (lane < l - l0) {
                const size_t pk = (size_t)pi * L + l0 + lane;
                uint8_t *o = nullptr;
                if (EMIT) {
                    o = a.out + a.pk_off[pk];
                    if (a.sop) {
                        const uint32_t ns = (uint32_t)(d.nsop0 + (l0 + lane) * (int)d.nsop_step) & 0xFFFFu;
                        o[0] = 0xFF; o[1] = 0x91; o[2] = 0; o[3] = 4; o[4] = (uint8_t)(ns >> 8); o[5] = (uint8_t)ns;
                        o += 6;
                    }
                }
                const uint32_t nbytes = stuff_header<EMIT>(buf, pws * 32u, pnb, o);
                if (EMIT) {
                    if (a.eph) { o[nbytes] = 0xFF; o[nbytes + 1] = 0x92; }
                    hdr = fixed + nbytes;
                } else {
                    a.pk_len[pk] = fixed + nbytes + pbody;
                }
            }
            if (EMIT)
                for (int l2 = l0; l2 < l; l2++) {
                    int n2 = 0, len2 = 0;
                    if (own) {
                        n2 = (int)S.nl[l2 * 64 + lane] - (l2 ? (int)S.nl[(l2 - 1) * 64 + lane] : 0);
                        len2 = S.lr[l2 * 64 + lane] - (l2 ? S.lr[(l2 - 1) * 64 + lane] : 0);
                    }
                    const uint32_t lin2 = n2 > 0 ? (uint32_t)len2 : 0u;
                    const uint32_t before = wave_incl_scan(lin2) - lin2;
                    const uint32_t h2 = (uint32_t)__builtin_amdgcn_readlane((int)hdr, l2 - l0);
                    const size_t pk2 = (size_t)pi * L + l2;
                    if (n2 > 0) a.blkdst[(size_t)b * L + l2] = a.pk_off[pk2] + h2 + before;
                }
            wave_lds_sync();
            for (uint32_t i = lane; i < used; i += 64) buf[i] = 0;
            wave_lds_sync();
            used = 0;
            l0 = l;
            if (l == L) break;
        }
        const uint32_t p = used * 32u;
        if (lane == 0 && nbits > 1) atomicOr(&buf[used], 0x80000000u);
        uint32_t q = p + 1u + off;
        lds_put_bits(buf, q, I, nI);
        q += (uint32_t)nI;
        lds_put_bits(buf, q, Z, nZ);
        q += (uint32_t)nZ;
        lds_put_bits(buf, q, p1v, p1n);
        q += (uint32_t)p1n;
        lds_put_bits(buf, q, (uint64_t)(uint32_t)len, p2n);
        if (lane == l - l0) {
            pws = used;
            pnb = nbits;
            pbody = body;
        }
        used += need;
    }
}

__device__ __forceinline__ int varint_len(uint32_t v) {
    int k = 1;
    while (v >>= 7) k++;
    return k;
}

struct RateStepArgs {
    RateState *rs;
    int64_t *budget;
    RateState *out_rs;
    T2Summary *out_sum;
};
template <bool SEQ>
__device__ __forceinline__ void seq_load8(const T2Args &a, size_t i0, size_t p1, size_t (&s8)[8]) {
#pragma unroll
    for (int j = 0; j < 8; j++) {
        const size_t i = min(i0 + j, p1 - 1);
        s8[j] = SEQ ? (size_t)a.seq[i] : i;
    }
}

template <bool SEQ>
__device__ __forceinline__ void tpart_size_seq(const T2Args &a, int t) {
    const TpDesc d = a.tps[t];
    const size_t p0 = (size_t)d.prec0 * a.L, p1 = (size_t)(d.prec0 + d.nprec) * a.L;
    uint64_t body = 0, plt = 0, seg = 0;
    for (size_t i0 = p0; i0 < p1; i0 += 8) {
        size_t s8[8];
        seq_load8<SEQ>(a, i0, p1, s8);
        uint32_t l8[8];
#pragma unroll
        for (int j = 0; j < 8; j++) l8[j] = a.pk_len[s8[j]];
#pragma unroll
        for (int j = 0; j < 8; j++) {
            const size_t i = i0 + j;
            if (i >= p1) break;
            const uint32_t len = l8[j];
            body += len;
            if (a.plt) {
                const uint64_t k = (uint64_t)varint_len(len);
                if (i == p0 || seg + k > 65532) {
                    if (i != p0) plt += 5 + seg;
                    seg = 0;
                }
                seg += k;
            }
        }
    }
    if (a.plt && p1 > p0) plt += 5 + seg;
    a.tp_hdr[t] = (uint32_t)(14 + plt);
    a.tp_len[t] = (uint32_t)(14 + plt + body);
}
__device__ __forceinline__ void tpart_size(const T2Args &a, int t) {
    if (a.seq) tpart_size_seq<true>(a, t);
    else tpart_size_seq<false>(a, t);
}

constexpr int kTotSums = kMaxLayers + 5;
struct T2TotalArgs {
    int nblocks;
    const int32_t *lengths;
    const uint8_t *npasses, *pmin;
    const int *t1err;
    const unsigned long long *pool_used;
    const uint64_t *kc;
    int ngroups;
    const unsigned long long *acc;
    T2Summary *sum;
    RateStepArgs rate;
    uint32_t *ticket;
};

template <int NT, bool T1>
__device__ __forceinline__ void t2_total_body(const T2Args &a, const T2TotalArgs &ta, uint64_t *wsum,
                                              int64_t (*red)[kTotSums]) {
    constexpr int NW = NT / 64;
    const int tid = threadIdx.x, lane = tid & 63, wv = tid >> 6;
    const int L = a.L;
    const int chunk = (a.ntp + NT - 1) / NT;
    const int t0 = min(a.ntp, tid * chunk), t1 = min(a.ntp, t0 + chunk);
    for (int t = t0; t < t1; t++) tpart_size(a, t);
    uint64_t s = 0, hdr = 0;
    for (int t = t0; t < t1; t++) s += a.tp_len[t];
    uint64_t tot;
    uint64_t o = wg_excl_scan64<NT>(s, wsum, tot);
    if (tid == 0) ta.sum->part_bytes = (int64_t)tot;
    for (int t = t0; t < t1; t++) {
        a.tp_off[t] = o;
        o += a.tp_len[t];
        hdr += a.tp_hdr[t];
    }
    int64_t lay[kMaxLayers];
#pragma unroll
    for (int l = 0; l < kMaxLayers; l++) lay[l] = 0;
    for (int pq = tid; pq < a.nprec; pq += NT) {
        const uint32_t *pl = a.pk_len + (size_t)pq * L;
#pragma unroll
        for (int l = 0; l < kMaxLayers; l++)
            if (l < L) lay[l] += pl[l];
    }
    int64_t tb = 0, tp = 0, nd = 0, skipped = 0;
    if (T1)
    for (int b0 = 0; b0 < ta.nblocks; b0 += 4 * NT) {
        int32_t ln[4];
        uint32_t np[4], pm[4];
        unsigned long long kk[4];
#pragma unroll
        for (int u = 0; u < 4; u++) {
            const int b = min(b0 + u * NT + tid, ta.nblocks - 1);
            ln[u] = ta.lengths[b];
            np[u] = ta.npasses[b];
            kk[u] = ta.acc[b];
            pm[u] = ta.pmin[b];
        }
#pragma unroll
        for (int u = 0; u < 4; u++)
            if (b0 + u * NT + tid < ta.nblocks) {
                tb += ln[u];
                tp += np[u];
                nd += (int64_t)(kk[u] & ((1ull << 40) - 1ull));
                skipped |= pm[u] > 0;
            }
    }
    auto wave_put = [&](int j, int64_t v) {
        v = wave_sum64(v);
        if (lane == 0) red[wv][j] = v;
    };
#pragma unroll
    for (int l = 0; l < kMaxLayers; l++)
        if (l < L) wave_put(l, lay[l]);
    wave_put(kMaxLayers + 0, (int64_t)hdr);
    if (T1) {
        wave_put(kMaxLayers + 1, tb);
        wave_put(kMaxLayers + 2, tp);
        wave_put(kMaxLayers + 3, nd);
        wave_put(kMaxLayers + 4, skipped);
    }
    __syncthreads();
    if (tid < (T1 ? kTotSums : kMaxLayers + 1) && (tid >= kMaxLayers || tid < L)) {
        int64_t v = 0;
#pragma unroll
        for (int w = 0; w < NW; w++) v += red[w][tid];
        if (tid < kMaxLayers) ta.sum->layer_bytes[tid] = v;
        else if (tid == kMaxLayers + 0) ta.sum->tp_hdr_bytes = v;
        else if (tid == kMaxLayers + 1) ta.sum->t1_bytes = v;
        else if (tid == kMaxLayers + 2) ta.sum->coded_passes = v;
        else if (tid == kMaxLayers + 3) ta.sum->decisions = v;
        else ta.sum->skipped = v != 0;
    }
    if (tid < L) {
        uint64_t k = 0;
        if (ta.kc)
            for (int g = 0; g < ta.ngroups; g++) k = max(k, ta.kc[(size_t)g * kMaxLayers + tid]);
        ta.sum->kc[tid] = k;
    }
    if (tid == 0) {
        ta.sum->err = *ta.t1err;
        ta.sum->stream_need = ta.pool_used ? (int64_t)*ta.pool_used : 0;
    }
    if (ta.rate.rs) {
        __syncthreads();
        if (tid == 0) rate_step(ta.rate.rs, ta.sum, L, ta.rate.budget, ta.rate.out_rs, ta.rate.out_sum);
    }
}

constexpr int kTotThreads = 1024, kTotWaves = kTotThreads / 64;
__global__ void __launch_bounds__(kTotThreads) k_t2_total(T2Args a, T2TotalArgs ta) {
    __shared__ uint64_t wsum[kTotWaves + 1];
    __shared__ int64_t red[kTotWaves][kTotSums];
    if (a.halt && *a.halt) return;
    t2_total_body<kTotThreads, true>(a, ta, wsum, red);
}

template <bool EMIT>
__global__ void __launch_bounds__(64 * kT2Waves) k_t2_wave(T2Args a, T2TotalArgs ta) {
    extern __shared__ __attribute__((aligned(16))) uint8_t t2dyn[];
    __shared__ uint64_t wsum[kT2Waves + 1];
    __shared__ int64_t red[kT2Waves][kTotSums];
    __shared__ int last;
    const int wv = threadIdx.x >> 6;
    const int pi = blockIdx.x * kT2Waves + wv;
    if (!EMIT && a.halt && *a.halt) return;
    if (pi < a.nprec) t2_wave_precinct<EMIT>(a, t2_lane(t2dyn, a.L, wv), pi);
    if (EMIT || !ta.ticket) return;
    asm volatile("s_waitcnt vmcnt(0)" ::: "memory");
    __syncthreads();
    if (threadIdx.x == 0) {
        __builtin_amdgcn_fence(__ATOMIC_RELEASE, "agent");
        asm volatile("s_waitcnt vmcnt(0)" ::: "memory");
        const uint32_t t = __hip_atomic_fetch_add(ta.ticket, 1u, __ATOMIC_RELAXED, __HIP_MEMORY_SCOPE_AGENT);
        last = t == gridDim.x - 1;
        if (last) {
            __builtin_amdgcn_fence(__ATOMIC_ACQUIRE, "agent");
            asm volatile("s_waitcnt vmcnt(0)" ::: "memory");
            *ta.ticket = 0u;
        }
    }
    __syncthreads();
    if (!last) return;
    t2_total_body<64 * kT2Waves, false>(a, ta, wsum, red);
}

template <bool SEQ>
__device__ __forceinline__ void tpart_emit(const T2Args &a, int t) {
    const TpDesc d = a.tps[t];
    uint8_t *p = a.out + a.base + a.tp_off[t];
    const uint32_t psot = a.tp_len[t];
    p[0] = 0xFF; p[1] = 0x90; p[2] = 0; p[3] = 10;
    p[4] = (uint8_t)(d.tile >> 8); p[5] = (uint8_t)d.tile;
    p[6] = (uint8_t)(psot >> 24); p[7] = (uint8_t)(psot >> 16); p[8] = (uint8_t)(psot >> 8); p[9] = (uint8_t)psot;
    p[10] = (uint8_t)d.tpsot;
    p[11] = (uint8_t)d.tnsot;
    p += 12;
    const size_t p0 = (size_t)d.prec0 * a.L, p1 = (size_t)(d.prec0 + d.nprec) * a.L;
    if (a.plt && p1 > p0) {
        size_t i = p0;
        int z = 0;
        uint8_t *hdr = p;
        p += 5;
        uint32_t seg = 0;
        while (i < p1) {
            size_t s8[8];
            seq_load8<SEQ>(a, i, p1, s8);
            uint32_t l8[8];
#pragma unroll
            for (int j = 0; j < 8; j++) l8[j] = a.pk_len[s8[j]];
#pragma unroll
            for (int j = 0; j < 8; j++) {
                if (i >= p1) break;
                const uint32_t len = l8[j];
                const int k = varint_len(len);
                if (seg + (uint32_t)k > 65532) {
                    hdr[0] = 0xFF; hdr[1] = 0x58;
                    hdr[2] = (uint8_t)((3 + seg) >> 8); hdr[3] = (uint8_t)(3 + seg);
                    hdr[4] = (uint8_t)z++;
                    hdr = p;
                    p += 5;
                    seg = 0;
                }
                for (int q = k - 1; q >= 0; q--) *p++ = (uint8_t)(((len >> (7 * q)) & 0x7F) | (q ? 0x80 : 0));
                seg += (uint32_t)k;
                i++;
            }
        }
        hdr[0] = 0xFF; hdr[1] = 0x58;
        hdr[2] = (uint8_t)((3 + seg) >> 8); hdr[3] = (uint8_t)(3 + seg);
        hdr[4] = (uint8_t)z;
    }
    p[0] = 0xFF; p[1] = 0x93;
    p += 2;
    uint64_t o = (uint64_t)(p - a.out);
    for (size_t i0 = p0; i0 < p1; i0 += 8) {
        size_t s8[8];
        seq_load8<SEQ>(a, i0, p1, s8);
        uint32_t l8[8];
#pragma unroll
        for (int j = 0; j < 8; j++) l8[j] = a.pk_len[s8[j]];
#pragma unroll
        for (int j = 0; j < 8; j++)
            if (i0 + j < p1) {
                a.pk_off[s8[j]] = o;
                o += l8[j];
            }
    }
}
__global__ void __launch_bounds__(64) k_t2_tp_emit(T2Args a) {
    const int t = blockIdx.x * 64 + threadIdx.x;
    if (t >= a.ntp) return;
    if (a.seq) tpart_emit<true>(a, t);
    else tpart_emit<false>(a, t);
}

__global__ void __launch_bounds__(256) k_t2_copy(T2Args a, int nblocks, const uint8_t *t1out) {
    const int b = blockIdx.x * 4 + (threadIdx.x >> 6), lane = threadIdx.x & 63;
    if (b >= nblocks) return;
    const int L = a.L;
    int r1 = 0, r0 = 0, np = 0, pp = 0;
    uint64_t dst = 0;
    if (lane < L) {
        r1 = a.lrate[(size_t)b * L + lane];
        np = a.nl[(size_t)b * L + lane];
        if (lane) {
            r0 = a.lrate[(size_t)b * L + lane - 1];
            pp = a.nl[(size_t)b * L + lane - 1];
        }
        dst = a.blkdst[(size_t)b * L + lane];
    }
    const uint64_t live = __ballot(lane < L && np > pp);
    const uint8_t *src0 = t1out + a.blocks[b].out_off;
    for (uint64_t m = live; m; m &= m - 1) {
        const int l = __builtin_ctzll(m);
        const int s0 = __builtin_amdgcn_readlane(r0, l);
        const int n = __builtin_amdgcn_readlane(r1, l) - s0;
        const uint8_t *s = src0 + s0;
        uint8_t *d = a.out + (((uint64_t)__builtin_amdgcn_readlane((uint32_t)(dst >> 32), l) << 32) |
                              (uint32_t)__builtin_amdgcn_readlane((uint32_t)dst, l));
        const int head = min(n, (int)((0u - (uint32_t)(uintptr_t)d) & 3u));
        if (lane < head) d[lane] = s[lane];
        const uint8_t *s4 = s + head;
        uint32_t *d4 = (uint32_t *)(d + head);
        const int nw = (n - head) >> 2;
        const uint32_t sh = (uint32_t)(uintptr_t)s4 & 3u;
        const uint32_t *sa = (const uint32_t *)(s4 - sh);
        for (int i = lane; i < nw; i += 64) d4[i] = __builtin_amdgcn_alignbyte(sa[i + 1], sa[i], sh);
        const int t0 = head + 4 * nw;
        if (lane < n - t0) d[t0 + lane] = s[t0 + lane];
    }
}

__global__ void __launch_bounds__(64) k_release_dma(int64_t *dep) {
    if (threadIdx.x == 0) __hip_atomic_store(dep, (int64_t)0, __ATOMIC_RELEASE, __HIP_MEMORY_SCOPE_SYSTEM);
}

#define HSACHECK(x)                                                                    \
    do {                                                                               \
        hsa_status_t s_ = (x);                                                         \
        if (s_ != HSA_STATUS_SUCCESS) {                                                \
            const char *m_ = "?";                                                      \
            hsa_status_string(s_, &m_);                                                \
            err = std::string(#x) + ": " + m_;                                         \
            return false;                                                              \
        }                                                                              \
    } while (0)

static uint64_t hsa_ticks(uint64_t ns) {
    static const uint64_t freq = [] {
        uint64_t f = 0;
        if (hsa_system_get_info(HSA_SYSTEM_INFO_TIMESTAMP_FREQUENCY, &f) != HSA_STATUS_SUCCESS || !f) f = 1000000000ull;
        return f;
    }();
    return (uint64_t)((double)ns * (double)freq / 1e9) + 1;
}

static uint64_t mono_ns() {
    return (uint64_t)std::chrono::duration_cast<std::chrono::nanoseconds>(
               std::chrono::steady_clock::now().time_since_epoch()).count();
}

static jp2hip::SliceResult poll_signal(hsa_signal_t sig, uint64_t slice_ns) {
    const hsa_signal_value_t v =
        hsa_signal_wait_scacquire(sig, HSA_SIGNAL_CONDITION_LT, 1, hsa_ticks(slice_ns), HSA_WAIT_STATE_BLOCKED);
    return v < 0 ? jp2hip::SliceResult::Error : (v < 1 ? jp2hip::SliceResult::Done : jp2hip::SliceResult::Pending);
}

static constexpr uint64_t kWaitSliceNs = 50ull * 1000 * 1000;
static constexpr uint64_t kDrainedGraceNs = 20ull * 1000 * 1000 * 1000;

static hsa_status_t first_cpu_agent(hsa_agent_t a, void *out) {
    hsa_device_type_t t;
    if (hsa_agent_get_info(a, HSA_AGENT_INFO_DEVICE, &t) == HSA_STATUS_SUCCESS && t == HSA_DEVICE_TYPE_CPU) {
        *(hsa_agent_t *)out = a;
        return HSA_STATUS_INFO_BREAK;
    }
    return HSA_STATUS_SUCCESS;
}

struct DmaGpu {
    std::mutex mu;
    bool probed = false;
    std::vector<int> fast;
    std::vector<std::pair<int, double>> rates;
    std::atomic<unsigned> next{0};
};
struct DmaEngines {
    std::mutex mu;
    std::map<uint64_t, std::unique_ptr<DmaGpu>> gpu;
};
static DmaEngines &dma_engines() {
    static DmaEngines *e = new DmaEngines();
    return *e;
}

static int pick_dma_engine(hsa_agent_t gpu, hsa_agent_t cpu, hsa_signal_t sig) {
    DmaEngines &E = dma_engines();
    DmaGpu *G;
    {
        std::lock_guard<std::mutex> lk(E.mu);
        std::unique_ptr<DmaGpu> &slot = E.gpu[gpu.handle];
        if (!slot) slot.reset(new DmaGpu());
        G = slot.get();
    }
    {
        std::lock_guard<std::mutex> lk(G->mu);
        if (!G->probed) {
            uint32_t mask = 0;
            const size_t n = 32u << 20;
            void *d = nullptr, *h = nullptr;
            if (hsa_amd_memory_copy_engine_status(cpu, gpu, &mask) == HSA_STATUS_SUCCESS && mask &&
                hipMalloc(&d, n) == hipSuccess && hipHostMalloc(&h, n, hipHostMallocDefault) == hipSuccess) {
                for (int e = 0; e < 16; e++) {
                    if (!(mask & (1u << e))) continue;
                    double best = 0.0;
                    for (int r = 0; r < 2; r++) {
                        hsa_signal_store_relaxed(sig, 1);
                        const auto t0 = std::chrono::steady_clock::now();
                        if (hsa_amd_memory_async_copy_on_engine(h, cpu, d, gpu, n, 0, nullptr, sig,
                                                                (hsa_amd_sdma_engine_id_t)(1u << e), true) != HSA_STATUS_SUCCESS)
                            break;
                        std::string perr;
                        if (!jp2hip::wait_bounded([&](uint64_t ns) { return poll_signal(sig, ns); },
                                                  [](std::string &) { return jp2hip::StreamState::Drained; }, mono_ns,
                                                  kWaitSliceNs, 1000ull * 1000 * 1000, "DMA engine probe", perr))
                            break;
                        const double sec = std::chrono::duration<double>(std::chrono::steady_clock::now() - t0).count();
                        best = std::max(best, n / sec);
                    }
                    if (best > 0.0) G->rates.emplace_back(e, best / 1e9);
                }
                double top = 0.0;
                for (auto &r : G->rates) top = std::max(top, r.second);
                for (auto &r : G->rates)
                    if (r.second >= 0.9 * top) G->fast.push_back(r.first);
            }
            if (d) (void)hipFree(d);
            if (h) (void)hipHostFree(h);
            G->probed = true;
        }
    }
    if (G->fast.empty()) return -1;
    return G->fast[(size_t)(G->next++) % G->fast.size()];
}

std::string dma_engine_report() {
    DmaEngines &E = dma_engines();
    std::lock_guard<std::mutex> lk(E.mu);
    std::string out;
    char buf[64];
    for (auto &kv : E.gpu) {
        DmaGpu &G = *kv.second;
        std::lock_guard<std::mutex> lg(G.mu);
        if (!G.probed) continue;
        if (!out.empty()) out += "; ";
        out += "agent " + std::to_string(kv.first) + ": using";
        for (int e : G.fast) out += " " + std::to_string(e);
        if (G.fast.empty()) out += " the runtime's choice";
        out += " of";
        for (auto &r : G.rates) {
            std::snprintf(buf, sizeof buf, " %d:%.1fGB/s", r.first, r.second);
            out += buf;
        }
    }
    return out;
}

bool GpuEncoder::dma_init(std::string &err) {
    if (dma_ok) return true;
    if (!t2out.ptr) {
        err = "dma_init: no device buffer yet";
        return false;
    }
    if (!hsa_up) {
        HSACHECK(hsa_init());
        hsa_up = true;
    }
    hsa_amd_pointer_info_t pi;
    std::memset(&pi, 0, sizeof pi);
    pi.size = sizeof pi;
    HSACHECK(hsa_amd_pointer_info(t2out.ptr, &pi, nullptr, nullptr, nullptr));
    dma_gpu = pi.agentOwner;
    if (hsa_iterate_agents(first_cpu_agent, &dma_cpu) != HSA_STATUS_INFO_BREAK) {
        err = "dma_init: no CPU agent";
        return false;
    }
    if (!dma_dep.handle) HSACHECK(hsa_amd_signal_create(1, 0, nullptr, HSA_AMD_SIGNAL_AMD_GPU_ONLY, &dma_dep));
    if (!dma_done.handle) HSACHECK(hsa_signal_create(1, 0, nullptr, &dma_done));
    HSACHECK(hsa_amd_signal_value_pointer(dma_dep, &dma_dep_val));
    dma_engine = pick_dma_engine(dma_gpu, dma_cpu, dma_done);
    dma_ok = true;
    return true;
}

bool GpuEncoder::dma_to_host(uint8_t *host_dst, const void *src, size_t bytes, std::string &err) {
    if (!dma_init(err)) return false;
    hsa_signal_store_relaxed(dma_dep, 1);
    hsa_signal_store_relaxed(dma_done, 1);
    hipLaunchKernelGGL(k_release_dma, dim3(1), dim3(64), 0, stream, (int64_t *)dma_dep_val);
    HIPCHECK(hipGetLastError());
    const hsa_status_t s =
        dma_engine >= 0
            ? hsa_amd_memory_async_copy_on_engine(host_dst, dma_cpu, src, dma_gpu, bytes, 1, &dma_dep, dma_done,
                                                  (hsa_amd_sdma_engine_id_t)(1u << dma_engine), true)
            : hsa_amd_memory_async_copy(host_dst, dma_cpu, src, dma_gpu, bytes, 1, &dma_dep, dma_done);
    if (s != HSA_STATUS_SUCCESS) {
        const char *m = "?";
        hsa_status_string(s, &m);
        std::string e2;
        (void)host_wait(e2);
        err = std::string("code-stream copy: hsa_amd_memory_async_copy: ") + m;
        return false;
    }
    waits++;
    hipStream_t st = stream;
    const bool ok = jp2hip::wait_bounded(
        [&](uint64_t ns) { return poll_signal(dma_done, ns); },
        [st](std::string &why) {
            const hipError_t q = hipStreamQuery(st);
            if (q == hipSuccess) return jp2hip::StreamState::Drained;
            if (q == hipErrorNotReady) return jp2hip::StreamState::Running;
            why = hipGetErrorString(q);
            return jp2hip::StreamState::Failed;
        },
        mono_ns, kWaitSliceNs, kDrainedGraceNs, "code-stream copy", err);
    if (!ok) {
        dma_dep.handle = 0;
        dma_done.handle = 0;
        dma_ok = false;
    }
    return ok;
}
T2Args GpuEncoder::t2_args(const Plan &plan) const {
    T2Args a;
    std::memset(&a, 0, sizeof a);
    a.prec = (const PrecDesc *)t2prec.ptr;
    a.nprec = t2_nprec;
    a.tps = (const TpDesc *)t2tp.ptr;
    a.ntp = t2_ntp;
    a.blocks = (const BlockDesc *)blocks.ptr;
    a.P = (const uint8_t *)P.ptr;
    a.nl = (uint8_t *)nl.ptr;
    a.lrate = (int32_t *)lrate.ptr;
    a.nhull = (const uint8_t *)nhull.ptr;
    a.hpass = (const uint8_t *)hpass.ptr;
    a.npasses = (const uint8_t *)npasses.ptr;
    a.hkey = (const uint64_t *)hkey.ptr;
    a.K = (const uint64_t *)thr.ptr;
    a.grp_b0 = (const int32_t *)grptab.ptr;
    a.ngroups = plan.ngroups();
    a.rates = (const int32_t *)rates.ptr;
    a.lossless = plan.rc.rate_bpp <= 0.0;
    a.L = plan.rc.layers;
    a.sop = plan.rc.sop;
    a.eph = plan.rc.eph;
    a.plt = plan.rc.plt;
    a.tt = (uint32_t *)t2tt.ptr;
    a.lblock = (int8_t *)t2lblock.ptr;
    a.incl = (int8_t *)t2incl.ptr;
    a.pk_len = (uint32_t *)t2pklen.ptr;
    a.seq = t2_seq ? (const uint32_t *)t2seq.ptr : nullptr;
    a.tp_len = (uint32_t *)t2tplen.ptr;
    a.tp_hdr = (uint32_t *)t2tphdr.ptr;
    a.tp_off = (uint64_t *)t2tpoff.ptr;
    a.pk_off = (uint64_t *)t2pkoff.ptr;
    a.blkdst = (uint64_t *)t2blkdst.ptr;
    a.out = (uint8_t *)t2out.ptr;
    return a;
}

bool GpuEncoder::t2_load(const Plan &plan, const T2Tables &T, std::string &err) {
    HIPCHECK(hipSetDevice(device));
    const int nb = (int)plan.blocks.size();
    const int L = plan.rc.layers;
    t2_nprec = (int)T.prec.size();
    t2_ntp = (int)T.tp.size();
    t2_seq = !T.seq.empty();
    int max_mb = 0;
    for (const BlockDesc &bd : plan.blocks) max_mb = std::max(max_mb, (int)bd.Mb);
    t2_wave = T.max_prec_blocks <= 64 && max_mb <= kWaveMaxMb;
    const size_t npk = (size_t)t2_nprec * L;
    if (!ensure<PrecDesc>(t2prec, T.prec.size(), err) || !ensure<TpDesc>(t2tp, T.tp.size(), err) ||
        !ensure<uint32_t>(t2tt, (size_t)T.tt_nodes, err) || !ensure<int8_t>(t2lblock, nb, err) ||
        !ensure<int8_t>(t2incl, nb, err) || !ensure<uint32_t>(t2pklen, npk, err) ||
        !ensure<uint64_t>(t2pkoff, npk, err) || !ensure<uint32_t>(t2tplen, T.tp.size(), err) ||
        !ensure<uint32_t>(t2tphdr, T.tp.size(), err) || !ensure<uint64_t>(t2tpoff, T.tp.size(), err) ||
        !ensure<uint64_t>(t2blkdst, (size_t)nb * L, err) || !ensure<T2Summary>(t2sum, 1, err) ||
        (t2_seq && !ensure<uint32_t>(t2seq, T.seq.size(), err)))
        return false;
    if (!h_sum) HIPCHECK(hipHostMalloc((void **)&h_sum, sizeof(T2Summary), hipHostMallocDefault));
    if (!t2ticket.ptr) {
        if (!ensure<uint32_t>(t2ticket, 1, err)) return false;
        HIPCHECK(hipMemsetAsync(t2ticket.ptr, 0, sizeof(uint32_t), stream));
    }
    if (plan.gen && plan.gen == t2_gen) {
        reuse |= JP2HIP_REUSED_T2_TABLES;
        return true;
    }
    t2_gen = 0;
    if (!h2d(t2prec.ptr, T.prec.data(), sizeof(PrecDesc) * T.prec.size(), err) ||
        !h2d(t2tp.ptr, T.tp.data(), sizeof(TpDesc) * T.tp.size(), err) ||
        (t2_seq && !h2d(t2seq.ptr, T.seq.data(), sizeof(uint32_t) * T.seq.size(), err)))
        return false;
    t2_gen = plan.gen;
    return true;
}

void GpuEncoder::t2_size_launch(const Plan &plan, bool with_kc, const int *halt, RateState *rs,
                                RateState *out_rs) {
    const int nb = (int)plan.blocks.size();
    T2Args a = t2_args(plan);
    a.halt = halt;
    RateStepArgs ra;
    ra.rs = rs;
    ra.budget = (int64_t *)budget.ptr;
    ra.out_rs = out_rs;
    ra.out_sum = out_rs ? (T2Summary *)(out_rs + 1) : nullptr;
    T2TotalArgs ta;
    ta.nblocks = nb;
    ta.lengths = (const int32_t *)lengths.ptr;
    ta.npasses = (const uint8_t *)npasses.ptr;
    ta.pmin = (const uint8_t *)pmin.ptr;
    ta.t1err = (const int *)this->err.ptr;
    ta.pool_used = mqspan.ptr ? (const unsigned long long *)mqspan.ptr + 2 : nullptr;
    ta.kc = with_kc ? (const uint64_t *)thr.ptr + (size_t)plan.ngroups() * kMaxLayers : (const uint64_t *)nullptr;
    ta.ngroups = plan.ngroups();
    ta.acc = (const unsigned long long *)ordkey.ptr;
    ta.sum = (T2Summary *)t2sum.ptr;
    ta.rate = ra;
    ta.ticket = nullptr;
    REPEAT_IF(5) {
        if (t2_nprec && t2_wave) {
            ta.ticket = (uint32_t *)t2ticket.ptr;
            hipLaunchKernelGGL(k_t2_wave<false>, dim3((t2_nprec + kT2Waves - 1) / kT2Waves), dim3(64 * kT2Waves),
                               kT2Waves * t2_lane_bytes(a.L), stream, a, ta);
        } else {
            ta.ticket = nullptr;
            if (t2_nprec) hipLaunchKernelGGL(k_t2_code<false>, dim3((t2_nprec + 63) / 64), dim3(64), 0, stream, a);
            hipLaunchKernelGGL(k_t2_total, dim3(1), dim3(kTotThreads), 0, stream, a, ta);
        }
    }
}

bool GpuEncoder::t2_size(const Plan &plan, bool with_kc, bool profile, StageTimes &st, T2Summary &sum,
                         std::string &err) {
    HIPCHECK(hipSetDevice(device));
    HIPCHECK(hipEventRecord(ev[kEvT2Begin], stream));
    t2_size_launch(plan, with_kc, nullptr);
    HIPCHECK(hipGetLastError());
    HIPCHECK(hipMemcpyAsync(h_sum, t2sum.ptr, sizeof(T2Summary), hipMemcpyDeviceToHost, stream));
    HIPCHECK(hipEventRecord(ev[kEvT2End], stream));
    if (!host_wait(err)) return false;
    sum = *h_sum;
    if (profile) {
        float t;
        HIPCHECK(hipEventElapsedTime(&t, ev[kEvSelectBegin], ev[kEvSelectEnd]));
        st.pcrd += t;
        HIPCHECK(hipEventElapsedTime(&t, ev[kEvT2Begin], ev[kEvT2End]));
        st.t2 += t;
    }
    return true;
}

bool GpuEncoder::t2_reserve(uint64_t part_bytes, std::string &err) {
    HIPCHECK(hipSetDevice(device));
    return ensure<uint8_t>(t2out, part_bytes, err);
}

bool GpuEncoder::t2_emit(const Plan &plan, uint64_t base, uint64_t part_bytes, uint8_t *host_dst, bool profile,
                         StageTimes &st, std::string &err) {
    HIPCHECK(hipSetDevice(device));
    const int nb = (int)plan.blocks.size();
    if (!ensure<uint8_t>(t2out, base + part_bytes, err)) return false;
    T2Args a = t2_args(plan);
    a.base = base;
    HIPCHECK(hipEventRecord(ev[kEvT2Begin], stream));
    if (t2_ntp) hipLaunchKernelGGL(k_t2_tp_emit, dim3((t2_ntp + 63) / 64), dim3(64), 0, stream, a);
    if (t2_nprec && t2_wave)
        hipLaunchKernelGGL(k_t2_wave<true>, dim3((t2_nprec + kT2Waves - 1) / kT2Waves), dim3(64 * kT2Waves),
                           kT2Waves * t2_lane_bytes(a.L), stream, a, T2TotalArgs{});
    else if (t2_nprec)
        hipLaunchKernelGGL(k_t2_code<true>, dim3((t2_nprec + 63) / 64), dim3(64), 0, stream, a);
    if (nb) hipLaunchKernelGGL(k_t2_copy, dim3((nb + 3) / 4), dim3(256), 0, stream, a, nb, (const uint8_t *)t1out.ptr);
    HIPCHECK(hipGetLastError());
#if defined(JP2HIP_DIAG_NO_D2H)
    HIPCHECK(hipEventRecord(ev[kEvT2End], stream));
    if (!host_wait(err)) return false;
    (void)host_dst;
#elif !defined(JP2HIP_D2H_BLIT)
    if (part_bytes) {
        if (!dma_to_host(host_dst, (const uint8_t *)t2out.ptr + base, part_bytes, err)) return false;
        HIPCHECK(hipEventRecord(ev[kEvT2End], stream));
        if (profile && !host_wait(err)) return false;
    } else {
        HIPCHECK(hipEventRecord(ev[kEvT2End], stream));
        if (!host_wait(err)) return false;
    }
#else
    if (part_bytes)
        HIPCHECK(hipMemcpyAsync(host_dst, (const uint8_t *)t2out.ptr + base, part_bytes, hipMemcpyDeviceToHost, stream));
    HIPCHECK(hipEventRecord(ev[kEvT2End], stream));
    if (!host_wait(err)) return false;
#endif
    if (profile) {
        float t;
        HIPCHECK(hipEventElapsedTime(&t, ev[kEvT2Begin], ev[kEvT2End]));
        st.d2h += t;
    }
    return true;
}

}
```

Baseline: 36440.

## Cache packet heads during sizing and emit tier-2 with a single fused kernel

The sizing pass of the wave tier-2 kernel now writes each stuffed packet header into a fixed per-precinct slot. It also records header lengths, packet offsets relative to their tile-part, and block offsets within each packet. The emit path no longer reruns the wave precinct coder. One combined kernel writes the tile-part headers, copies the cached heads and copies code-block bodies with aligned word copies. This adds head-slot memory, new host tables and an overflow error code, and the PLT length loops now prefetch the next group of eight entries.

```diff
diff --git a/jp2-bucketeer_amd/csrc/encode.cpp b/jp2-bucketeer_amd/csrc/encode.cpp
--- a/jp2-bucketeer_amd/csrc/encode.cpp
+++ b/jp2-bucketeer_amd/csrc/encode.cpp
@@ -194,7 +194,7 @@
             }
             break;
         }
-        if (sum.err) return fail("tier-1 output capacity exceeded");
+        if (sum.err) return fail(device_err_text(sum.err));
         iters = 1;
         cs_bytes = (int64_t)mh_bytes + sum.part_bytes + 2;
     } else {
@@ -216,7 +216,7 @@
                 restart = true;
                 continue;
             }
-            if (sum.err) return fail("tier-1 output capacity exceeded");
+            if (sum.err) return fail(device_err_text(sum.err));
             if (rs.safety) {
                 init.skip_target = -1;
                 if (!ctx->gpu.run_front(d_src, *lay, plan, prof, st, err, -1)) return fail(err);
@@ -332,7 +332,7 @@
                   ctx->gpu.t2_size(sub, lossless, prof, st, sum, err);
         if (rok && have && sum.err) {
             rok = false;
-            err = "tier-1 output capacity exceeded";
+            err = device_err_text(sum.err);
         }
         std::vector<int64_t> v((size_t)L + 3 + (lossless ? (size_t)world * L : 0), 0);
         if (rok && have) {
diff --git a/jp2-bucketeer_amd/csrc/gpu_encoder.cpp b/jp2-bucketeer_amd/csrc/gpu_encoder.cpp
--- a/jp2-bucketeer_amd/csrc/gpu_encoder.cpp
+++ b/jp2-bucketeer_amd/csrc/gpu_encoder.cpp
@@ -113,7 +113,7 @@
         err = "context on device " + std::to_string(device) + ": its stream is on device " + std::to_string((int)sd);
         return false;
     }
-    const DevBuf *bufs[] = {&src, &coef, &bp, &t1out, &stream_buf, &t2out, &blocks};
+    const DevBuf *bufs[] = {&src, &coef, &bp, &t1out, &stream_buf, &t2out, &t2heads, &blocks};
     for (const DevBuf *b : bufs) {
         if (!b->ptr) continue;
         hipPointerAttribute_t at;
diff --git a/jp2-bucketeer_amd/csrc/gpu_encoder.h b/jp2-bucketeer_amd/csrc/gpu_encoder.h
--- a/jp2-bucketeer_amd/csrc/gpu_encoder.h
+++ b/jp2-bucketeer_amd/csrc/gpu_encoder.h
@@ -45,6 +45,9 @@
                                                                            \
     X(hdist) X(rstate) X(t2ticket) X(t2prec) X(t2tp) X(t2tt) X(t2lblock) X(t2incl) X(t2pklen) X(t2pkoff)      \
     X(t2tplen) X(t2tphdr) X(t2tpoff) X(t2blkdst) X(t2out) X(t2sum) X(t2seq)                                   \
+              \
+                    \
+    X(t2pemit) X(t2blkprec) X(t2heads) X(t2pkhlen) X(t2pkrel) X(t2blkrel)                                     \
                \
     X(expanded) X(exoff) X(exlut)
 
diff --git a/jp2-bucketeer_amd/csrc/jp2hip_internal.h b/jp2-bucketeer_amd/csrc/jp2hip_internal.h
--- a/jp2-bucketeer_amd/csrc/jp2hip_internal.h
+++ b/jp2-bucketeer_amd/csrc/jp2hip_internal.h
@@ -33,6 +33,10 @@
 QuantTab quant_tab(const jp2hip_recipe &rc, int bits);
 
 constexpr int kErrSlotPool = 8;
+constexpr int kErrT2Head = 16;
+inline const char *device_err_text(int e) {
+    return (e & kErrT2Head) ? "tier-2 packet head exceeds its slot" : "tier-1 output capacity exceeded";
+}
 
 struct BlockDesc {
     int32_t tc;
@@ -118,9 +122,25 @@
     int32_t tile, tpsot, tnsot;
     int32_t prec0, nprec;
 };
+constexpr int kWaveMaxMb = 48;
+constexpr uint32_t head_bits_bound(int nblocks, int L) {
+    return 1u + (uint32_t)nblocks * (uint32_t)((L + 7) + (kWaveMaxMb + 7) + (16 + 28 + 1) + 38);
+}
+constexpr uint32_t head_slot_bytes(int nblocks, int L, bool sop, bool eph) {
+    return ((sop ? 6u : 0u) + (eph ? 2u : 0u) + (head_bits_bound(nblocks, L) + 6u) / 7u + 1u + 3u) & ~3u;
+}
+struct PrecEmit {
+    uint64_t hd_off;
+    uint32_t slot;
+    int32_t tp;
+};
+static_assert(sizeof(PrecEmit) == 16, "PrecEmit layout");
 struct T2Tables {
     std::vector<PrecDesc> prec;
     std::vector<TpDesc> tp;
+    std::vector<PrecEmit> pemit;
+    std::vector<int32_t> blk_prec;
+    uint64_t head_bytes = 0;
     std::vector<uint32_t> seq;
     int64_t tt_nodes = 0;
     int max_prec_blocks = 0;
diff --git a/jp2-bucketeer_amd/csrc/t2.cpp b/jp2-bucketeer_amd/csrc/t2.cpp
--- a/jp2-bucketeer_amd/csrc/t2.cpp
+++ b/jp2-bucketeer_amd/csrc/t2.cpp
@@ -171,6 +171,9 @@
     T.prec.clear();
     T.tp.clear();
     T.seq.clear();
+    T.pemit.clear();
+    T.blk_prec.clear();
+    T.head_bytes = 0;
     T.tt_nodes = 0;
     T.max_prec_blocks = 0;
     std::vector<std::vector<TpDesc>> per_tile((size_t)std::max(0, tile1 - tile0));
@@ -204,6 +207,18 @@
                             if (pb.ncw && pb.nch) T.tt_nodes += 2 * tree_nodes(pb.ncw, pb.nch);
                         }
                         T.max_prec_blocks = std::max(T.max_prec_blocks, blocks);
+                        PrecEmit pe;
+                        pe.hd_off = T.head_bytes;
+                        pe.slot = blocks <= 64 ? head_slot_bytes(blocks, L, rc.sop != 0, rc.eph != 0) : 0u;
+                        pe.tp = 0;
+                        T.head_bytes += (uint64_t)L * pe.slot;
+                        for (int bi = 0; bi < pr.nb; bi++)
+                            for (int k = 0; k < pr.pb[bi].ncw * pr.pb[bi].nch; k++) {
+                                const size_t b = (size_t)(d.first[bi] + k);
+                                if (b >= T.blk_prec.size()) T.blk_prec.resize(b + 1, -1);
+                                T.blk_prec[b] = (int32_t)T.prec.size();
+                            }
+                        T.pemit.push_back(pe);
                         T.prec.push_back(d);
                         tp.nprec++;
                         nsop += L;
@@ -234,6 +249,8 @@
             }
         ty0 = e;
     }
+    for (size_t ti = 0; ti < T.tp.size(); ti++)
+        for (int32_t p = T.tp[ti].prec0; p < T.tp[ti].prec0 + T.tp[ti].nprec; p++) T.pemit[(size_t)p].tp = (int32_t)ti;
 }
 
 
diff --git a/jp2-bucketeer_amd/csrc/t2_device.hip b/jp2-bucketeer_amd/csrc/t2_device.hip
--- a/jp2-bucketeer_amd/csrc/t2_device.hip
+++ b/jp2-bucketeer_amd/csrc/t2_device.hip
@@ -44,6 +44,13 @@
     uint64_t *tp_off;
     uint64_t *pk_off;
     uint64_t *blkdst;
+    const PrecEmit *pemit;
+    const int32_t *blk_prec;
+    uint8_t *heads;
+    uint32_t *pk_hlen;
+    uint32_t *pk_rel;
+    uint32_t *blkrel;
+    int *err;
     uint8_t *out;
     uint64_t base;
     const int *halt;
@@ -271,7 +278,7 @@
 constexpr int kT2Waves = 4;
 constexpr int kTreeLev = 7;
 constexpr int kBitWords = 512;
-constexpr int kWaveMaxMb = 48;
+static_assert(head_bits_bound(64, kMaxLayers) + 32 <= kBitWords * 32, "kBitWords");
 struct T2LaneShared {
     int32_t *lr;
     uint32_t *bits;
@@ -306,30 +313,41 @@
     if (w2) atomicOr(w + 2, w2);
 }
 
-template <bool EMIT>
-__device__ __forceinline__ uint32_t stuff_header(const uint32_t *buf, uint32_t p0, uint32_t nbits, uint8_t *o) {
-    uint32_t q = 0, nbytes = 0, byte = 0;
+struct HeadOut {
+    uint32_t *w;
+    uint32_t acc, n;
+    __device__ __forceinline__ void init(uint8_t *slot) { w = (uint32_t *)slot; acc = 0; n = 0; }
+    __device__ __forceinline__ void put(uint32_t byte) {
+        acc |= byte << (8u * (n & 3u));
+        n++;
+        if (!(n & 3u)) {
+            if (w) w[(n >> 2) - 1u] = acc;
+            acc = 0;
+        }
+    }
+    __device__ __forceinline__ void finish() {
+        if (w && (n & 3u)) w[n >> 2] = acc;
+    }
+};
+
+__device__ __forceinline__ void stuff_header(const uint32_t *buf, uint32_t p0, uint32_t nbits, HeadOut &o) {
+    uint32_t q = 0, byte = 0;
     int cap = 8;
     while (q < nbits) {
         const uint32_t p = p0 + q;
         const uint64_t win = ((uint64_t)buf[p >> 5] << 32) | buf[(p >> 5) + 1];
         byte = (uint32_t)(win >> (64 - cap - (int)(p & 31u))) & ((1u << cap) - 1u);
-        if (EMIT) o[nbytes] = (uint8_t)byte;
-        nbytes++;
+        o.put(byte);
         q += (uint32_t)cap;
         cap = byte == 0xFFu ? 7 : 8;
     }
-    if (byte == 0xFFu) {
-        if (EMIT) o[nbytes] = 0;
-        nbytes++;
-    }
-    return nbytes;
-}
-
-template <bool EMIT>
+    if (byte == 0xFFu) o.put(0);
+}
+
 __device__ __forceinline__ void t2_wave_precinct(const T2Args &a, const T2LaneShared &S, int pi) {
     const int lane = threadIdx.x & 63;
     const PrecDesc d = a.prec[pi];
+    const PrecEmit pe = a.pemit[pi];
     const int L = a.L;
     const int c0 = d.nb > 0 ? d.ncw[0] * d.nch[0] : 0, c1 = d.nb > 1 ? d.ncw[1] * d.nch[1] : 0,
               c2 = d.nb > 2 ? d.ncw[2] * d.nch[2] : 0;
@@ -346,7 +364,7 @@
         zero_planes = a.blocks[b].Mb - a.P[b];
         uint8_t *gnl = a.nl + (size_t)b * L;
         int32_t *glr = a.lrate + (size_t)b * L;
-        if (!EMIT) {
+        {
             const int nh = a.nhull[b];
             const uint8_t *hp = a.hpass + (size_t)b * (kMaxPasses + 1);
             const uint64_t *hk = a.hkey + (size_t)b * (kMaxPasses + 1);
@@ -393,11 +411,6 @@
                     gnl[l] = (uint8_t)ncv[j];
                     glr[l] = r;
                 }
-            }
-        } else {
-            for (int l = 0; l < L; l++) {
-                S.nl[l * 64 + lane] = gnl[l];
-                S.lr[l * 64 + lane] = glr[l];
             }
         }
     }
@@ -504,45 +517,30 @@
             off = wave_incl_scan(T) - T;
             nbits = 1u + (uint32_t)__shfl((int)(off + T), 63, 64);
             const uint32_t lin = n > 0 ? (uint32_t)len : 0u;
-            body = (uint32_t)__shfl((int)wave_incl_scan(lin), 63, 64);
+            const uint32_t upto = wave_incl_scan(lin);
+            if (n > 0) a.blkrel[(size_t)b * L + l] = upto - lin;
+            body = (uint32_t)__shfl((int)upto, 63, 64);
             need = (nbits + 31u) / 32u + 1u;
             if (!nonempty) nbits = 1;
         }
         if (l == L || used + need > (uint32_t)kBitWords) {
             wave_lds_sync();
-            uint32_t hdr = 0;
             if (lane < l - l0) {
                 const size_t pk = (size_t)pi * L + l0 + lane;
-                uint8_t *o = nullptr;
-                if (EMIT) {
-                    o = a.out + a.pk_off[pk];
-                    if (a.sop) {
-                        const uint32_t ns = (uint32_t)(d.nsop0 + (l0 + lane) * (int)d.nsop_step) & 0xFFFFu;
-                        o[0] = 0xFF; o[1] = 0x91; o[2] = 0; o[3] = 4; o[4] = (uint8_t)(ns >> 8); o[5] = (uint8_t)ns;
-                        o += 6;
-                    }
+                const bool fits = fixed + (pnb + 6u) / 7u + 1u <= pe.slot;
+                if (!fits) atomicOr(a.err, kErrT2Head);
+                HeadOut o;
+                o.init(fits ? a.heads + pe.hd_off + (size_t)(l0 + lane) * pe.slot : nullptr);
+                if (a.sop) {
+                    const uint32_t ns = (uint32_t)(d.nsop0 + (l0 + lane) * (int)d.nsop_step) & 0xFFFFu;
+                    o.put(0xFF); o.put(0x91); o.put(0); o.put(4); o.put(ns >> 8); o.put(ns & 0xFFu);
                 }
-                const uint32_t nbytes = stuff_header<EMIT>(buf, pws * 32u, pnb, o);
-                if (EMIT) {
-                    if (a.eph) { o[nbytes] = 0xFF; o[nbytes + 1] = 0x92; }
-                    hdr = fixed + nbytes;
-                } else {
-                    a.pk_len[pk] = fixed + nbytes + pbody;
-                }
-            }
-            if (EMIT)
-                for (int l2 = l0; l2 < l; l2++) {
-                    int n2 = 0, len2 = 0;
-                    if (own) {
-                        n2 = (int)S.nl[l2 * 64 + lane] - (l2 ? (int)S.nl[(l2 - 1) * 64 + lane] : 0);
-                        len2 = S.lr[l2 * 64 + lane] - (l2 ? S.lr[(l2 - 1) * 64 + lane] : 0);
-                    }
-                    const uint32_t lin2 = n2 > 0 ? (uint32_t)len2 : 0u;
-                    const uint32_t before = wave_incl_scan(lin2) - lin2;
-                    const uint32_t h2 = (uint32_t)__builtin_amdgcn_readlane((int)hdr, l2 - l0);
-                    const size_t pk2 = (size_t)pi * L + l2;
-                    if (n2 > 0) a.blkdst[(size_t)b * L + l2] = a.pk_off[pk2] + h2 + before;
-                }
+                stuff_header(buf, pws * 32u, pnb, o);
+                if (a.eph) { o.put(0xFF); o.put(0x92); }
+                o.finish();
+                a.pk_hlen[pk] = o.n;
+                a.pk_len[pk] = o.n + pbody;
+            }
             wave_lds_sync();
             for (uint32_t i = lane; i < used; i += 64) buf[i] = 0;
             wave_lds_sync();
@@ -591,21 +589,28 @@
 }
 
 template <bool SEQ>
+__device__ __forceinline__ void len_load8(const T2Args &a, size_t i0, size_t p1, size_t (&s8)[8], uint32_t (&l8)[8]) {
+    seq_load8<SEQ>(a, i0, p1, s8);
+#pragma unroll
+    for (int j = 0; j < 8; j++) l8[j] = a.pk_len[s8[j]];
+}
+
+template <bool SEQ>
 __device__ __forceinline__ void tpart_size_seq(const T2Args &a, int t) {
     const TpDesc d = a.tps[t];
     const size_t p0 = (size_t)d.prec0 * a.L, p1 = (size_t)(d.prec0 + d.nprec) * a.L;
     uint64_t body = 0, plt = 0, seg = 0;
+    size_t s8[8], sn[8] = {};
+    uint32_t l8[8], ln[8] = {};
+    if (p1 > p0) len_load8<SEQ>(a, p0, p1, s8, l8);
     for (size_t i0 = p0; i0 < p1; i0 += 8) {
-        size_t s8[8];
-        seq_load8<SEQ>(a, i0, p1, s8);
-        uint32_t l8[8];
-#pragma unroll
-        for (int j = 0; j < 8; j++) l8[j] = a.pk_len[s8[j]];
+        if (i0 + 8 < p1) len_load8<SEQ>(a, i0 + 8, p1, sn, ln);
 #pragma unroll
         for (int j = 0; j < 8; j++) {
             const size_t i = i0 + j;
             if (i >= p1) break;
             const uint32_t len = l8[j];
+            if (a.pk_rel) a.pk_rel[s8[j]] = (uint32_t)body;
             body += len;
             if (a.plt) {
                 const uint64_t k = (uint64_t)varint_len(len);
@@ -615,6 +620,11 @@
                 }
                 seg += k;
             }
+        }
+#pragma unroll
+        for (int j = 0; j < 8; j++) {
+            s8[j] = sn[j];
+            l8[j] = ln[j];
         }
     }
     if (a.plt && p1 > p0) plt += 5 + seg;
@@ -742,7 +752,6 @@
     t2_total_body<kTotThreads, true>(a, ta, wsum, red);
 }
 
-template <bool EMIT>
 __global__ void __launch_bounds__(64 * kT2Waves) k_t2_wave(T2Args a, T2TotalArgs ta) {
     extern __shared__ __attribute__((aligned(16))) uint8_t t2dyn[];
     __shared__ uint64_t wsum[kT2Waves + 1];
@@ -750,9 +759,8 @@
     __shared__ int last;
     const int wv = threadIdx.x >> 6;
     const int pi = blockIdx.x * kT2Waves + wv;
-    if (!EMIT && a.halt && *a.halt) return;
-    if (pi < a.nprec) t2_wave_precinct<EMIT>(a, t2_lane(t2dyn, a.L, wv), pi);
-    if (EMIT || !ta.ticket) return;
+    if (a.halt && *a.halt) return;
+    if (pi < a.nprec) t2_wave_precinct(a, t2_lane(t2dyn, a.L, wv), pi);
     asm volatile("s_waitcnt vmcnt(0)" ::: "memory");
     __syncthreads();
     if (threadIdx.x == 0) {
@@ -772,7 +780,7 @@
 }
 
 template <bool SEQ>
-__device__ __forceinline__ void tpart_emit(const T2Args &a, int t) {
+__device__ __forceinline__ uint8_t *tpart_header(const T2Args &a, int t) {
     const TpDesc d = a.tps[t];
     uint8_t *p = a.out + a.base + a.tp_off[t];
     const uint32_t psot = a.tp_len[t];
@@ -789,12 +797,11 @@
         uint8_t *hdr = p;
         p += 5;
         uint32_t seg = 0;
+        size_t s8[8], sn[8] = {};
+        uint32_t l8[8], ln[8] = {};
+        len_load8<SEQ>(a, i, p1, s8, l8);
         while (i < p1) {
-            size_t s8[8];
-            seq_load8<SEQ>(a, i, p1, s8);
-            uint32_t l8[8];
-#pragma unroll
-            for (int j = 0; j < 8; j++) l8[j] = a.pk_len[s8[j]];
+            if (i + 8 < p1) len_load8<SEQ>(a, i + 8, p1, sn, ln);
 #pragma unroll
             for (int j = 0; j < 8; j++) {
                 if (i >= p1) break;
@@ -812,14 +819,25 @@
                 seg += (uint32_t)k;
                 i++;
             }
+#pragma unroll
+            for (int j = 0; j < 8; j++) {
+                s8[j] = sn[j];
+                l8[j] = ln[j];
+            }
         }
         hdr[0] = 0xFF; hdr[1] = 0x58;
         hdr[2] = (uint8_t)((3 + seg) >> 8); hdr[3] = (uint8_t)(3 + seg);
         hdr[4] = (uint8_t)z;
     }
     p[0] = 0xFF; p[1] = 0x93;
-    p += 2;
-    uint64_t o = (uint64_t)(p - a.out);
+    return p + 2;
+}
+
+template <bool SEQ>
+__device__ __forceinline__ void tpart_emit(const T2Args &a, int t) {
+    const TpDesc d = a.tps[t];
+    const size_t p0 = (size_t)d.prec0 * a.L, p1 = (size_t)(d.prec0 + d.nprec) * a.L;
+    uint64_t o = (uint64_t)(tpart_header<SEQ>(a, t) - a.out);
     for (size_t i0 = p0; i0 < p1; i0 += 8) {
         size_t s8[8];
         seq_load8<SEQ>(a, i0, p1, s8);
@@ -839,6 +857,19 @@
     if (t >= a.ntp) return;
     if (a.seq) tpart_emit<true>(a, t);
     else tpart_emit<false>(a, t);
+}
+
+__device__ __forceinline__ void wave_copy_piece(uint8_t *d, const uint8_t *s, int n, int lane) {
+    const int head = min(n, (int)((0u - (uint32_t)(uintptr_t)d) & 3u));
+    if (lane < head) d[lane] = s[lane];
+    const uint8_t *s4 = s + head;
+    uint32_t *d4 = (uint32_t *)(d + head);
+    const int nw = (n - head) >> 2;
+    const uint32_t sh = (uint32_t)(uintptr_t)s4 & 3u;
+    const uint32_t *sa = (const uint32_t *)(s4 - sh);
+    for (int i = lane; i < nw; i += 64) d4[i] = __builtin_amdgcn_alignbyte(sa[i + 1], sa[i], sh);
+    const int t0 = head + 4 * nw;
+    if (lane < n - t0) d[t0 + lane] = s[t0 + lane];
 }
 
 __global__ void __launch_bounds__(256) k_t2_copy(T2Args a, int nblocks, const uint8_t *t1out) {
@@ -862,19 +893,80 @@
         const int l = __builtin_ctzll(m);
         const int s0 = __builtin_amdgcn_readlane(r0, l);
         const int n = __builtin_amdgcn_readlane(r1, l) - s0;
-        const uint8_t *s = src0 + s0;
         uint8_t *d = a.out + (((uint64_t)__builtin_amdgcn_readlane((uint32_t)(dst >> 32), l) << 32) |
                               (uint32_t)__builtin_amdgcn_readlane((uint32_t)dst, l));
-        const int head = min(n, (int)((0u - (uint32_t)(uintptr_t)d) & 3u));
-        if (lane < head) d[lane] = s[lane];
-        const uint8_t *s4 = s + head;
-        uint32_t *d4 = (uint32_t *)(d + head);
-        const int nw = (n - head) >> 2;
-        const uint32_t sh = (uint32_t)(uintptr_t)s4 & 3u;
-        const uint32_t *sa = (const uint32_t *)(s4 - sh);
-        for (int i = lane; i < nw; i += 64) d4[i] = __builtin_amdgcn_alignbyte(sa[i + 1], sa[i], sh);
-        const int t0 = head + 4 * nw;
-        if (lane < n - t0) d[t0 + lane] = s[t0 + lane];
+        wave_copy_piece(d, src0 + s0, n, lane);
+    }
+}
+
+constexpr int kEmitThreads = 256, kEmitWaves = kEmitThreads / 64;
+struct T2EmitGrid {
+    int tp_wgs, head_wgs, body_wgs;
+    int nblocks;
+    const uint8_t *t1out;
+};
+
+__device__ __forceinline__ uint64_t packet_start(const T2Args &a, int pi, int lane) {
+    const int t = a.pemit[pi].tp;
+    return a.base + a.tp_off[t] + a.tp_hdr[t] + a.pk_rel[(size_t)pi * a.L + lane];
+}
+
+__global__ void __launch_bounds__(kEmitThreads) k_t2_emit(T2Args a, T2EmitGrid g) {
+    const int lane = threadIdx.x & 63, wv = threadIdx.x >> 6;
+    const int L = a.L;
+    int wg = blockIdx.x;
+    if (wg < g.tp_wgs) {
+        const int t = wg * kEmitThreads + threadIdx.x;
+        if (t >= a.ntp) return;
+        if (a.seq) (void)tpart_header<true>(a, t);
+        else (void)tpart_header<false>(a, t);
+        return;
+    }
+    wg -= g.tp_wgs;
+    if (wg < g.head_wgs) {
+        const int pi = wg * kEmitWaves + wv;
+        if (pi >= a.nprec) return;
+        const PrecEmit pe = a.pemit[pi];
+        uint32_t hl = 0;
+        uint64_t at = 0;
+        if (lane < L) {
+            hl = a.pk_hlen[(size_t)pi * L + lane];
+            at = packet_start(a, pi, lane);
+        }
+        const uint8_t *src = a.heads + pe.hd_off;
+        for (int l = 0; l < L; l++) {
+            const uint32_t n = min((uint32_t)__builtin_amdgcn_readlane((int)hl, l), pe.slot);
+            uint8_t *d = a.out + (((uint64_t)__builtin_amdgcn_readlane((uint32_t)(at >> 32), l) << 32) |
+                                  (uint32_t)__builtin_amdgcn_readlane((uint32_t)at, l));
+            for (uint32_t i = lane; i < n; i += 64) d[i] = src[(size_t)l * pe.slot + i];
+        }
+        return;
+    }
+    wg -= g.head_wgs;
+    const int b = wg * kEmitWaves + wv;
+    if (b >= g.nblocks) return;
+    int r1 = 0, r0 = 0, np = 0, pp = 0;
+    uint64_t dst = 0;
+    if (lane < L) {
+        const int pi = a.blk_prec[b];
+        r1 = a.lrate[(size_t)b * L + lane];
+        np = a.nl[(size_t)b * L + lane];
+        if (lane) {
+            r0 = a.lrate[(size_t)b * L + lane - 1];
+            pp = a.nl[(size_t)b * L + lane - 1];
+        }
+        if (np > pp)
+            dst = packet_start(a, pi, lane) + a.pk_hlen[(size_t)pi * L + lane] + a.blkrel[(size_t)b * L + lane];
+    }
+    const uint64_t live = __ballot(lane < L && np > pp);
+    const uint8_t *src0 = g.t1out + a.blocks[b].out_off;
+    for (uint64_t m = live; m; m &= m - 1) {
+        const int l = __builtin_ctzll(m);
+        const int s0 = __builtin_amdgcn_readlane(r0, l);
+        const int n = __builtin_amdgcn_readlane(r1, l) - s0;
+        uint8_t *d = a.out + (((uint64_t)__builtin_amdgcn_readlane((uint32_t)(dst >> 32), l) << 32) |
+                              (uint32_t)__builtin_amdgcn_readlane((uint32_t)dst, l));
+        wave_copy_piece(d, src0 + s0, n, lane);
     }
 }
 
@@ -1110,8 +1202,18 @@
     a.tp_len = (uint32_t *)t2tplen.ptr;
     a.tp_hdr = (uint32_t *)t2tphdr.ptr;
     a.tp_off = (uint64_t *)t2tpoff.ptr;
-    a.pk_off = (uint64_t *)t2pkoff.ptr;
-    a.blkdst = (uint64_t *)t2blkdst.ptr;
+    if (t2_wave) {
+        a.pemit = (const PrecEmit *)t2pemit.ptr;
+        a.blk_prec = (const int32_t *)t2blkprec.ptr;
+        a.heads = (uint8_t *)t2heads.ptr;
+        a.pk_hlen = (uint32_t *)t2pkhlen.ptr;
+        a.pk_rel = (uint32_t *)t2pkrel.ptr;
+        a.blkrel = (uint32_t *)t2blkrel.ptr;
+    } else {
+        a.pk_off = (uint64_t *)t2pkoff.ptr;
+        a.blkdst = (uint64_t *)t2blkdst.ptr;
+    }
+    a.err = (int *)err.ptr;
     a.out = (uint8_t *)t2out.ptr;
     return a;
 }
@@ -1130,11 +1232,35 @@
     if (!ensure<PrecDesc>(t2prec, T.prec.size(), err) || !ensure<TpDesc>(t2tp, T.tp.size(), err) ||
         !ensure<uint32_t>(t2tt, (size_t)T.tt_nodes, err) || !ensure<int8_t>(t2lblock, nb, err) ||
         !ensure<int8_t>(t2incl, nb, err) || !ensure<uint32_t>(t2pklen, npk, err) ||
-        !ensure<uint64_t>(t2pkoff, npk, err) || !ensure<uint32_t>(t2tplen, T.tp.size(), err) ||
+        !ensure<uint32_t>(t2tplen, T.tp.size(), err) ||
         !ensure<uint32_t>(t2tphdr, T.tp.size(), err) || !ensure<uint64_t>(t2tpoff, T.tp.size(), err) ||
-        !ensure<uint64_t>(t2blkdst, (size_t)nb * L, err) || !ensure<T2Summary>(t2sum, 1, err) ||
+        !ensure<T2Summary>(t2sum, 1, err) ||
         (t2_seq && !ensure<uint32_t>(t2seq, T.seq.size(), err)))
         return false;
+    if (t2_wave) {
+        if (T.pemit.size() != T.prec.size() || T.blk_prec.size() != (size_t)nb ||
+            std::find(T.blk_prec.begin(), T.blk_prec.end(), -1) != T.blk_prec.end()) {
+            err = "tier-2 tables: emission tables do not match the plan";
+            return false;
+        }
+        for (size_t i = 0; i < T.prec.size(); i++) {
+            const PrecDesc &d = T.prec[i];
+            int blk = 0;
+            for (int bi = 0; bi < d.nb; bi++) blk += (int)d.ncw[bi] * (int)d.nch[bi];
+            if (L > kMaxLayers || blk > 64 ||
+                T.pemit[i].slot < head_slot_bytes(blk, L, plan.rc.sop != 0, plan.rc.eph != 0) ||
+                T.pemit[i].hd_off + (uint64_t)L * T.pemit[i].slot > T.head_bytes) {
+                err = "tier-2 tables: a packet head slot is below the header bound";
+                return false;
+            }
+        }
+        if (!ensure<PrecEmit>(t2pemit, T.pemit.size(), err) || !ensure<int32_t>(t2blkprec, nb, err) ||
+            !ensure<uint8_t>(t2heads, (size_t)T.head_bytes, err) || !ensure<uint32_t>(t2pkhlen, npk, err) ||
+            !ensure<uint32_t>(t2pkrel, npk, err) || !ensure<uint32_t>(t2blkrel, (size_t)nb * L, err))
+            return false;
+    } else if (!ensure<uint64_t>(t2pkoff, npk, err) || !ensure<uint64_t>(t2blkdst, (size_t)nb * L, err)) {
+        return false;
+    }
     if (!h_sum) HIPCHECK(hipHostMalloc((void **)&h_sum, sizeof(T2Summary), hipHostMallocDefault));
     if (!t2ticket.ptr) {
         if (!ensure<uint32_t>(t2ticket, 1, err)) return false;
@@ -1147,7 +1273,9 @@
     t2_gen = 0;
     if (!h2d(t2prec.ptr, T.prec.data(), sizeof(PrecDesc) * T.prec.size(), err) ||
         !h2d(t2tp.ptr, T.tp.data(), sizeof(TpDesc) * T.tp.size(), err) ||
-        (t2_seq && !h2d(t2seq.ptr, T.seq.data(), sizeof(uint32_t) * T.seq.size(), err)))
+        (t2_seq && !h2d(t2seq.ptr, T.seq.data(), sizeof(uint32_t) * T.seq.size(), err)) ||
+        (t2_wave && (!h2d(t2pemit.ptr, T.pemit.data(), sizeof(PrecEmit) * T.pemit.size(), err) ||
+                     !h2d(t2blkprec.ptr, T.blk_prec.data(), sizeof(int32_t) * T.blk_prec.size(), err))))
         return false;
     t2_gen = plan.gen;
     return true;
@@ -1179,7 +1307,7 @@
     REPEAT_IF(5) {
         if (t2_nprec && t2_wave) {
             ta.ticket = (uint32_t *)t2ticket.ptr;
-            hipLaunchKernelGGL(k_t2_wave<false>, dim3((t2_nprec + kT2Waves - 1) / kT2Waves), dim3(64 * kT2Waves),
+            hipLaunchKernelGGL(k_t2_wave, dim3((t2_nprec + kT2Waves - 1) / kT2Waves), dim3(64 * kT2Waves),
                                kT2Waves * t2_lane_bytes(a.L), stream, a, ta);
         } else {
             ta.ticket = nullptr;
@@ -1222,13 +1350,20 @@
     T2Args a = t2_args(plan);
     a.base = base;
     HIPCHECK(hipEventRecord(ev[kEvT2Begin], stream));
-    if (t2_ntp) hipLaunchKernelGGL(k_t2_tp_emit, dim3((t2_ntp + 63) / 64), dim3(64), 0, stream, a);
-    if (t2_nprec && t2_wave)
-        hipLaunchKernelGGL(k_t2_wave<true>, dim3((t2_nprec + kT2Waves - 1) / kT2Waves), dim3(64 * kT2Waves),
-                           kT2Waves * t2_lane_bytes(a.L), stream, a, T2TotalArgs{});
-    else if (t2_nprec)
-        hipLaunchKernelGGL(k_t2_code<true>, dim3((t2_nprec + 63) / 64), dim3(64), 0, stream, a);
-    if (nb) hipLaunchKernelGGL(k_t2_copy, dim3((nb + 3) / 4), dim3(256), 0, stream, a, nb, (const uint8_t *)t1out.ptr);
+    if (t2_wave) {
+        T2EmitGrid g;
+        g.tp_wgs = (t2_ntp + kEmitThreads - 1) / kEmitThreads;
+        g.head_wgs = (t2_nprec + kEmitWaves - 1) / kEmitWaves;
+        g.body_wgs = t2_nprec ? (nb + kEmitWaves - 1) / kEmitWaves : 0;
+        g.nblocks = nb;
+        g.t1out = (const uint8_t *)t1out.ptr;
+        const int wgs = g.tp_wgs + g.head_wgs + g.body_wgs;
+        if (wgs) hipLaunchKernelGGL(k_t2_emit, dim3(wgs), dim3(kEmitThreads), 0, stream, a, g);
+    } else {
+        if (t2_ntp) hipLaunchKernelGGL(k_t2_tp_emit, dim3((t2_ntp + 63) / 64), dim3(64), 0, stream, a);
+        if (t2_nprec) hipLaunchKernelGGL(k_t2_code<true>, dim3((t2_nprec + 63) / 64), dim3(64), 0, stream, a);
+        if (nb) hipLaunchKernelGGL(k_t2_copy, dim3((nb + 3) / 4), dim3(256), 0, stream, a, nb, (const uint8_t *)t1out.ptr);
+    }
     HIPCHECK(hipGetLastError());
 #if defined(JP2HIP_DIAG_NO_D2H)
     HIPCHECK(hipEventRecord(ev[kEvT2End], stream));
```

Result: no change. 36160 (-0.8%).
